# julienperriercornet/turbosqueeze

Hardware: AMD Instinct MI355X
Metric: encode+decode GB/s on enwik9-shaped input (round trip of uncompressed bytes) (higher is better)
Workload: dtype u8

## Files before the change

### turbosqueeze_amd/csrc/tsq_dec_common.cuh

```cuda
#pragma once

#include <type_traits>

#include "tsq_common.cuh"

namespace tsq {

#ifdef TSQ_STATS
__device__ unsigned long long g_dec_stats[16];
__device__ unsigned long long g_dec_wave[48];
#define TSQD_T0() unsigned long long t0_ = __builtin_amdgcn_s_memtime()
#define TSQD_ACC(slot) do { unsigned long long t1_ = __builtin_amdgcn_s_memtime(); st_[slot] += t1_ - t0_; t0_ = t1_; } while (0)
#define TSQD_CNT(slot, v) st_[slot] += (v)
#else
#define TSQD_T0() do {} while (0)
#define TSQD_ACC(slot) do {} while (0)
#define TSQD_CNT(slot, v) do {} while (0)
#endif

struct SymCfg {
    static constexpr uint32_t T = 1024;
    static constexpr uint32_t S = 6144;
    static constexpr uint32_t SPAD = 160;
    static constexpr uint32_t OUTC = 2 * S;
    static constexpr uint32_t HOP = 16;
    static constexpr uint32_t MAXG = 512;
    static constexpr uint32_t MAXSN = MAXG / HOP + 2;
    static constexpr uint32_t PER = S / T;
    static constexpr uint32_t TERM = S + SPAD;
    static constexpr uint32_t R = 65536 + OUTC + 64;
    static constexpr uint32_t RPAD = 64;
    static constexpr uint32_t SWORDS = (S + SPAD + 16) / 16;
};
static_assert(SymCfg::R % 16 == 0, "ring phase");
static_assert(SymCfg::OUTC == 12 * SymCfg::T, "twelve bytes per lane");
static_assert(SymCfg::S % SymCfg::T == 0 && SymCfg::SWORDS <= SymCfg::T, "lane counts");
static_assert(SymCfg::MAXG <= SymCfg::T / 2 && SymCfg::MAXG % SymCfg::HOP == 0 && SymCfg::MAXG >= SymCfg::S / 13 + 2 * SymCfg::HOP, "group table");
static_assert(4 * SymCfg::MAXG <= 2 * SymCfg::T, "at most two pairs per lane");

__device__ __forceinline__ void pair_lens(uint32_t sb, uint32_t cc, uint32_t ext, uint32_t& slen, uint32_t& olen)
{
    const uint32_t hi = sb >> 4, lo = sb & 15u;
    const uint32_t lit_hi = cc & 2u, lit_lo = cc & 1u;
    const uint32_t o_hi = (!lit_hi && ext && hi < 3u) ? (hi + 2u) << 4 : hi + 1u;
    const uint32_t o_lo = (!lit_lo && ext && lo < 3u) ? (lo + 2u) << 4 : lo + 1u;
    slen = 1u + (lit_hi ? hi + 1u : 2u) + (lit_lo ? lo + 1u : 2u);
    olen = o_hi + o_lo;
}

struct Image {
    uint32_t op, len, at;
    __device__ __forceinline__ uint32_t lead() const { return at & 3u; }
    __device__ __forceinline__ uint32_t a0() const { return at & ~3u; }
};

__device__ __forceinline__ uint4 prefetch_words(const uint8_t* in, uint32_t at, uint32_t av)
{
    using C = SymCfg;
    const uint32_t tid = threadIdx.x;
    const uint32_t lim = av < C::S + C::SPAD ? av : C::S + C::SPAD;
    uint4 w = make_uint4(0, 0, 0, 0);
    if (tid < C::SWORDS && (tid << 4) + 16u <= lim) __builtin_memcpy(&w, in + at + (tid << 4), 16);
    return w;
}
template <class L>
__device__ __forceinline__ void stage_words(uint8_t* lds, const uint8_t* in, uint32_t at, uint32_t av, uint4 pre)
{
    using C = SymCfg;
    const uint32_t tid = threadIdx.x;
    if (tid < C::SWORDS) {
        uint4 w = pre;
        const uint32_t lim = av < C::S + C::SPAD ? av : C::S + C::SPAD, o = tid << 4;
        if (o < lim && o + 16u > lim) {
            uint32_t b[4] = {0, 0, 0, 0};
            for (uint32_t k = 0; o + k < lim; ++k) b[k >> 2] |= (uint32_t)in[at + o + k] << (8u * (k & 3u));
            w = make_uint4(b[0], b[1], b[2], b[3]);
        }
        *reinterpret_cast<uint4*>(lds + L::sbuf + (tid << 4)) = w;
    }
}

template <class L>
__device__ __forceinline__ void parse_groups(uint8_t* lds, uint32_t slim, uint32_t (&x)[SymCfg::PER])
{
    using C = SymCfg;
    const uint32_t tid = threadIdx.x;
    const uint8_t* const sbuf = lds + L::sbuf;
    uint32_t y[C::PER], c[C::PER];
    {
        uint32_t* const pl = reinterpret_cast<uint32_t*>(lds + L::j4);
        constexpr uint32_t NW = (C::S + C::SPAD) / 4u;
#pragma unroll
        for (uint32_t k = 0; k < (NW + C::T - 1u) / C::T; ++k) {
            const uint32_t w = tid + k * C::T;
            if (w < NW) {
                const uint32_t v = reinterpret_cast<const uint32_t*>(sbuf)[w];
                uint32_t q[4];
#pragma unroll
                for (uint32_t b = 0; b < 4; ++b) {
                    const uint32_t hi = (v >> (8u * b + 4u)) & 15u, lo = (v >> (8u * b)) & 15u;
                    q[b] = 0x03040405u + (lo << 8) + (hi << 16) + ((lo + hi) << 24);
                }
                *reinterpret_cast<uint4*>(pl + 4u * w) = make_uint4(q[0], q[1], q[2], q[3]);
            }
        }
    }
    __syncthreads();
    {
        const uint32_t* const pl = reinterpret_cast<const uint32_t*>(lds + L::j4);
#pragma unroll
        for (uint32_t k = 0; k < C::PER; ++k) { const uint32_t o = tid + k * C::T; c[k] = (uint32_t)sbuf[o] << 3; x[k] = o + 1u; }
#pragma unroll
        for (uint32_t pr = 0; pr < 4; ++pr) {
#pragma unroll
            for (uint32_t k = 0; k < C::PER; ++k) y[k] = pl[x[k]];
#pragma unroll
            for (uint32_t k = 0; k < C::PER; ++k) x[k] += __builtin_amdgcn_ubfe(y[k], (c[k] >> (6u - 2u * pr)) & 0x18u, 8u);
        }
    }
    uint8_t* const j1 = lds + L::j1;
#pragma unroll
    for (uint32_t k = 0; k < C::PER; ++k) { const uint32_t o = tid + k * C::T; j1[o] = (uint8_t)(x[k] - o); x[k] = o < slim ? x[k] : C::TERM; }
    __syncthreads();
}

template <class L>
__device__ __forceinline__ void double_pointers(uint8_t* lds, uint32_t slim, uint32_t (&x)[SymCfg::PER])
{
    using C = SymCfg;
    const uint32_t tid = threadIdx.x;
    const uint8_t* const j1 = lds + L::j1;
    uint16_t* const j2 = reinterpret_cast<uint16_t*>(lds + L::j2);
    uint16_t* const j4 = reinterpret_cast<uint16_t*>(lds + L::j4);
    uint16_t* const j8 = reinterpret_cast<uint16_t*>(lds + L::j8);
    uint16_t* const j16 = reinterpret_cast<uint16_t*>(lds + L::j16);
    uint32_t y[C::PER];
#pragma unroll
    for (uint32_t k = 0; k < C::PER; ++k) { const uint32_t a = x[k] < slim ? x[k] : 0u; y[k] = a + j1[a]; }
#pragma unroll
    for (uint32_t k = 0; k < C::PER; ++k) { x[k] = x[k] < slim ? y[k] : C::TERM; j2[tid + k * C::T] = (uint16_t)x[k]; }
    if (tid <= C::SPAD) { j2[C::S + tid] = (uint16_t)C::TERM; j4[C::S + tid] = (uint16_t)C::TERM; j8[C::S + tid] = (uint16_t)C::TERM; j16[C::S + tid] = (uint16_t)C::TERM; }
    __syncthreads();
    const uint16_t* src = j2;
    uint16_t* const dsts[3] = {j4, j8, j16};
#pragma unroll
    for (uint32_t d = 0; d < 3; ++d) {
#pragma unroll
        for (uint32_t k = 0; k < C::PER; ++k) y[k] = src[x[k]];
#pragma unroll
        for (uint32_t k = 0; k < C::PER; ++k) { x[k] = y[k]; dsts[d][tid + k * C::T] = (uint16_t)x[k]; }
        __syncthreads();
        src = dsts[d];
    }
}

template <class L>
__device__ __forceinline__ uint32_t walk_chain(uint8_t* lds, uint32_t first, uint32_t slim)
{
    using C = SymCfg;
    const uint16_t* const j16 = reinterpret_cast<const uint16_t*>(lds + L::j16);
    uint16_t* const sn = reinterpret_cast<uint16_t*>(lds + L::sn);
    uint32_t* const misc = reinterpret_cast<uint32_t*>(lds + L::misc);
    if (threadIdx.x < 64u) {
        uint32_t x = first, k = 0;
        while (x < slim && k < C::MAXSN) {
            const uint32_t x1 = j16[x];
            const uint32_t x2 = j16[x1];
            sn[k++] = (uint16_t)x;
            if (x1 < slim && k < C::MAXSN) { sn[k++] = (uint16_t)x1; x = x2; }
            else x = x1;
        }
        if (threadIdx.x == 0) { misc[0] = k; if (k >= C::MAXSN && x < slim) misc[4] = kErrStream; }
    }
    __syncthreads();
    return misc[0];
}

template <class L>
__device__ __forceinline__ void group_lanes(uint8_t* lds, uint32_t nsn, uint32_t slim, uint32_t op, uint32_t size, uint32_t ext)
{
    using C = SymCfg;
    const uint32_t tid = threadIdx.x, lane = tid & 63u, wid = tid >> 6;
    const uint8_t* const sbuf = lds + L::sbuf;
    const uint8_t* const j1 = lds + L::j1;
    const uint16_t* const j2 = reinterpret_cast<const uint16_t*>(lds + L::j2);
    const uint16_t* const j4 = reinterpret_cast<const uint16_t*>(lds + L::j4);
    const uint16_t* const j8 = reinterpret_cast<const uint16_t*>(lds + L::j8);
    const uint16_t* const sn = reinterpret_cast<const uint16_t*>(lds + L::sn);
    uint16_t* const gstart = reinterpret_cast<uint16_t*>(lds + L::gstart);
    uint16_t* const glen = reinterpret_cast<uint16_t*>(lds + L::glen);
    uint32_t* const gout = reinterpret_cast<uint32_t*>(lds + L::gout);
    uint32_t* const pairs = reinterpret_cast<uint32_t*>(lds + L::pairs);
    uint32_t* const wsum = reinterpret_cast<uint32_t*>(lds + L::wsum);
    uint32_t* const misc = reinterpret_cast<uint32_t*>(lds + L::misc);
    uint32_t x = C::TERM;
    if (tid < nsn * C::HOP) {
        x = sn[tid >> 4];
        if (tid & 8u) x = j8[x];
        if (tid & 4u) x = j4[x];
        if (tid & 2u) x = j2[x];
        if (tid & 1u) x = x < slim ? (uint32_t)(x + j1[x]) : C::TERM;
    }
    uint32_t v = 0;
    if (x < slim) {
        gstart[tid] = (uint16_t)x;
        const uint32_t c = sbuf[x];
        uint32_t p = x + 1u, pw[4];
#pragma unroll
        for (uint32_t pr = 0; pr < 4; ++pr) {
            const uint32_t cc = (c >> (6u - 2u * pr)) & 3u;
            pw[pr] = p | (v << 13) | (cc << 30);
            uint32_t sl, ol;
            pair_lens(sbuf[p], cc, ext, sl, ol);
            p += sl;
            v += ol;
        }
        *reinterpret_cast<uint4*>(pairs + tid * 4u) = make_uint4(pw[0], pw[1], pw[2], pw[3]);
        glen[tid] = (uint16_t)v;
        if (p >= slim) { misc[1] = tid + 1u; misc[5] = p; }
    }
    const uint32_t incl = wave_scan_add(v);
    if (lane == 63) wsum[wid] = incl;
    __syncthreads();
    const uint32_t totals = wave_scan_add(lane < C::T / 64u ? wsum[lane] : 0u);
    const uint32_t before = wid ? (uint32_t)__builtin_amdgcn_readlane((int)totals, (int)wid - 1) : 0u;
    const uint32_t excl = before + incl - v;
    if (x < slim) {
        gout[tid] = op + excl;
        if (excl + 512u + 16u > C::OUTC) atomicMin(&misc[2], tid);
        if (op + excl + v >= size) atomicMin(&misc[3], tid);
    }
}

struct ChunkEnd {
    uint32_t ng;
    uint32_t next_at;
    uint32_t next_op;
    bool last;
    bool cut;
};
template <class L>
__device__ __forceinline__ ChunkEnd chunk_end(const uint8_t* lds, uint32_t op, uint32_t size)
{
    const uint16_t* const gstart = reinterpret_cast<const uint16_t*>(lds + L::gstart);
    const uint16_t* const glen = reinterpret_cast<const uint16_t*>(lds + L::glen);
    const uint32_t* const gout = reinterpret_cast<const uint32_t*>(lds + L::gout);
    const uint32_t* const misc = reinterpret_cast<const uint32_t*>(lds + L::misc);
    const uint32_t ng = misc[1], cut = misc[2], fin = misc[3];
    if (fin != 0xFFFFFFFFu && fin < cut) return {fin + 1u, 0u, size, true, false};
    if (cut != 0xFFFFFFFFu) return {cut, gstart[cut], gout[cut], false, true};
    return {ng, misc[5], ng ? gout[ng - 1] + glen[ng - 1] : op, false, false};
}

template <class L>
__device__ __forceinline__ void clear_records(uint8_t* lds)
{
    uint32_t* const recw = reinterpret_cast<uint32_t*>(lds + L::recw);
    for (uint32_t w = threadIdx.x; w < (SymCfg::OUTC + 16) / 4; w += SymCfg::T) *reinterpret_cast<uint4*>(recw + 4u * w) = make_uint4(0, 0, 0, 0);
}
template <class L, class PairAt>
__device__ __forceinline__ void drop_records(uint8_t* lds, uint32_t ng, const Image& im, uint32_t size, uint32_t avail, uint32_t ext,
                                             PairAt pair_at)
{
    using C = SymCfg;
    const uint32_t tid = threadIdx.x;
    const uint8_t* const sbuf = lds + L::sbuf;
    uint32_t* const recw = reinterpret_cast<uint32_t*>(lds + L::recw);
    const uint32_t op = im.op, lead = im.lead(), a0 = im.a0();
    if (tid == 0 && lead) recw[0] = 0x40000000u | (L::ring + a0);
    uint32_t bad = 0;
#pragma unroll
    for (uint32_t rep = 0; rep < 2; ++rep) {
        const uint32_t gi = tid + rep * C::T;
        if (gi >= ng * 4u) break;
        const uint2 pg = pair_at(rep, gi);
        const uint32_t pw = pg.x;
        uint32_t p = pw & 0x1FFFu, j = pg.y + ((pw >> 13) & 0x3FFFu);
        const uint32_t origin = j;
        uint32_t sb = 0;
        if (j < size) { if (p >= avail) bad = 1; sb = sbuf[p]; p++; }
#pragma unroll
        for (uint32_t sidx = 0; sidx < 2; ++sidx) {
            if (j < size && !bad) {
                const uint32_t nib = sidx == 0 ? sb >> 4 : sb & 15u;
                const uint32_t lit = (pw >> (31u - sidx)) & 1u;
                const uint32_t room = size - j;
                const uint32_t ij = j - op + lead;
                if (lit) {
                    const uint32_t len = nib + 1u, take = len < room ? len : room;
                    if (p + take > avail) bad = 1;
                    else recw[ij] = 0x40000000u | ((L::sbuf + p - ij) & 0xFFFFFFu);
                    p += len; j += take;
                } else {
                    if (p + 2u > avail) bad = 1;
                    const uint32_t off = (uint32_t)sbuf[p] | ((uint32_t)sbuf[p + 1] << 8);
                    p += 2;
                    const uint32_t len = ext ? nibble_span(nib) : nib + 1u;
                    const uint32_t take = len < room ? len : room;
                    if (off > origin || take > off) bad = 1;
                    if (!bad) {
                        const uint32_t a = origin - off;
                        const uint32_t n_hist = a >= op ? 0u : (op - a < take ? op - a : take);
                        if (n_hist) {
                            uint32_t x0 = a0 + C::R - ((op - a) - lead);
                            x0 -= x0 >= C::R ? C::R : 0u;
                            recw[ij] = 0x40000000u | ((L::ring + x0 - ij) & 0xFFFFFFu);
                            if (x0 + n_hist > C::R) { const uint32_t n1 = C::R - x0; recw[ij + n1] = 0x40000000u | ((L::ring - (ij + n1)) & 0xFFFFFFu); }
                        }
                        if (n_hist < take) recw[ij + n_hist] = 0xC0000000u | ((a - j) & 0xFFFFFFu);
                    }
                    j += take;
                }
            }
        }
    }
    if (bad) reinterpret_cast<uint32_t*>(lds + L::misc)[4] = kErrStream;
}

typedef __attribute__((address_space(3))) uint16_t lds_u16;

template <class L>
__device__ __forceinline__ uint32_t fetch_bytes(uint8_t* lds, const Image& im)
{
    const uint32_t tid = threadIdx.x, lane = tid & 63u, wid = tid >> 6;
    const uint32_t* const recw = reinterpret_cast<const uint32_t*>(lds + L::recw);
    uint32_t* const wsum = reinterpret_cast<uint32_t*>(lds + L::wsum);
    lds_u16* const wl = (lds_u16*)(lds + L::plist) + 768u * wid;
    const uint32_t own = 12u * tid;
    uint32_t r[12];
    {
        const uint4 q0 = *reinterpret_cast<const uint4*>(recw + own), q1 = *reinterpret_cast<const uint4*>(recw + own + 4u),
                    q2 = *reinterpret_cast<const uint4*>(recw + own + 8u);
        r[0] = q0.x; r[1] = q0.y; r[2] = q0.z; r[3] = q0.w; r[4] = q1.x; r[5] = q1.y; r[6] = q1.z; r[7] = q1.w; r[8] = q2.x; r[9] = q2.y; r[10] = q2.z; r[11] = q2.w;
#pragma unroll
        for (uint32_t k = 1; k < 12; ++k) r[k] = r[k] ? r[k] : r[k - 1];
        const uint32_t upto = wave_scan_last(r[11]);
        uint32_t carry = (uint32_t)__builtin_amdgcn_update_dpp(0, (int)upto, 0x138, 0xF, 0xF, false);
        if (lane == 63) wsum[wid] = upto;
        __syncthreads();
        {
            const uint32_t ws = lane < 16u ? wsum[lane] : 0u;
            const uint64_t m = __ballot(ws != 0u && lane < wid);
            const uint32_t prev = m ? (uint32_t)__builtin_amdgcn_readlane((int)ws, 63 - __builtin_clzll(m)) : 0u;
            carry = carry ? carry : prev;
        }
#pragma unroll
        for (uint32_t k = 0; k < 12; ++k) r[k] = r[k] ? r[k] : carry;
    }
    uint32_t pend = 0;
    if (own < im.lead() + im.len) {
        uint32_t v[12], by[12];
#pragma unroll
        for (uint32_t k = 0; k < 12; ++k) {
            v[k] = own + k + (uint32_t)((int32_t)(r[k] << 8) >> 8);
            pend |= (r[k] >> 31) << k;
        }
#pragma unroll
        for (uint32_t k = 0; k < 12; ++k) by[k] = lds[(r[k] >> 31) ? 0u : v[k]];
#pragma unroll
        for (uint32_t k = 0; k < 12; ++k) v[k] = (r[k] >> 31) ? v[k] : (0x8000u | by[k]);
#pragma unroll
        for (uint32_t w = 0; w < 3; ++w)
            *reinterpret_cast<uint2*>(lds + L::ent + 2u * own + 8u * w) = make_uint2(v[4 * w] | (v[4 * w + 1] << 16), v[4 * w + 2] | (v[4 * w + 3] << 16));
    }
    const uint32_t cnt = (uint32_t)__builtin_popcount(pend);
    const uint32_t incl = wave_scan_add(cnt);
    const uint32_t n_wait = (uint32_t)__builtin_amdgcn_readlane((int)incl, 63);
    uint32_t at = incl - cnt;
#pragma unroll
    for (uint32_t k = 0; k < 12; ++k) {
        if ((pend >> k) & 1u) wl[at] = (uint16_t)(own + k);
        at += (pend >> k) & 1u;
    }
    return n_wait;
}

template <class L>
__device__ __forceinline__ uint32_t jump_pointers(uint8_t* lds, uint32_t n_wait)
{
    const uint32_t lane = threadIdx.x & 63u, wid = threadIdx.x >> 6;
    lds_u16* const le = (lds_u16*)(lds + L::ent);
    lds_u16* const wl = (lds_u16*)(lds + L::plist) + 768u * wid;
    const uint32_t spare = SymCfg::OUTC + wid;
    if (lane == 0) le[spare] = 0x8000u;
    const uint32_t passes = (n_wait + 63u) >> 6;
    const uint32_t padded = passes <= 2u ? 2u : passes <= 4u ? 4u : passes <= 6u ? 6u : passes <= 8u ? 8u : 12u;
    if (passes) for (uint32_t it = n_wait + lane; it < padded * 64u; it += 64u) wl[it] = (uint16_t)spare;
    uint32_t iters = 0;
    auto jump = [&](auto passes_c) {
        constexpr uint32_t P = decltype(passes_c)::value;
        uint32_t q[P], ptr[P];
#pragma unroll
        for (uint32_t ps = 0; ps < P; ++ps) q[ps] = wl[ps * 64u + lane];
#pragma unroll
        for (uint32_t ps = 0; ps < P; ++ps) ptr[ps] = __hip_atomic_load(&le[q[ps]], __ATOMIC_RELAXED, __HIP_MEMORY_SCOPE_WORKGROUP);
        for (;;) {
            uint32_t e[P], open = 0;
#pragma unroll
            for (uint32_t ps = 0; ps < P; ++ps) e[ps] = __hip_atomic_load(&le[(ptr[ps] & 0x8000u) ? q[ps] : ptr[ps]], __ATOMIC_RELAXED, __HIP_MEMORY_SCOPE_WORKGROUP);
#pragma unroll
            for (uint32_t ps = 0; ps < P; ++ps) {
                __hip_atomic_store(&le[q[ps]], (uint16_t)e[ps], __ATOMIC_RELAXED, __HIP_MEMORY_SCOPE_WORKGROUP);
                ptr[ps] = e[ps];
                open |= (e[ps] & 0x8000u) ^ 0x8000u;
            }
            iters++;
            if (__ballot(open != 0u) == 0ull) break;
        }
    };
    if (passes == 0u) {}
    else if (passes <= 2u) jump(std::integral_constant<uint32_t, 2>{});
    else if (passes <= 4u) jump(std::integral_constant<uint32_t, 4>{});
    else if (passes <= 6u) jump(std::integral_constant<uint32_t, 6>{});
    else if (passes <= 8u) jump(std::integral_constant<uint32_t, 8>{});
    else jump(std::integral_constant<uint32_t, 12>{});
    return iters;
}

template <class L>
__device__ __forceinline__ void write_ring(uint8_t* lds, const Image& im)
{
    using C = SymCfg;
    const uint32_t own = 12u * threadIdx.x;
    if (own >= im.lead() + im.len) return;
    const uint2 e0 = *reinterpret_cast<const uint2*>(lds + L::ent + 2u * own), e1 = *reinterpret_cast<const uint2*>(lds + L::ent + 2u * own + 8u),
                e2 = *reinterpret_cast<const uint2*>(lds + L::ent + 2u * own + 16u);
    const uint32_t ev[6] = {e0.x, e0.y, e1.x, e1.y, e2.x, e2.y};
#pragma unroll
    for (uint32_t w = 0; w < 3; ++w) {
        uint32_t x = im.a0() + own + 4u * w; x -= x >= C::R ? C::R : 0u;
        const uint32_t lo = ev[2 * w], hi = ev[2 * w + 1];
        *reinterpret_cast<uint32_t*>(lds + L::ring + x) = (lo & 0xFFu) | ((lo >> 8) & 0xFF00u) | ((hi & 0xFFu) << 16) | ((hi >> 16) << 24);
    }
}

template <class L>
__device__ __forceinline__ void flush_image(const uint8_t* lds, uint8_t* out, const Image& im, uint32_t first_tid, uint32_t n_threads)
{
    using C = SymCfg;
    const uint32_t tid = threadIdx.x;
    const uint8_t* const ring = lds + L::ring;
    if (im.len == 0 || tid < first_tid) return;
    const uint32_t t = tid - first_tid;
    const uint32_t head = (16u - (im.at & 15u)) & 15u;
    const uint32_t hb = head < im.len ? head : im.len;
    if (t < hb) out[im.op + t] = ring[im.at + t];
    const uint32_t words = (im.len - hb) >> 4;
    uint32_t ra = im.at + hb; ra -= ra >= C::R ? C::R : 0u;
    for (uint32_t w = t; w < words; w += n_threads) {
        uint32_t a = ra + (w << 4); a -= a >= C::R ? C::R : 0u;
        *reinterpret_cast<uint4*>(out + im.op + hb + (w << 4)) = *reinterpret_cast<const uint4*>(ring + a);
    }
    const uint32_t tail_at = hb + (words << 4);
    if (t < im.len - tail_at) { uint32_t a = ra + (words << 4) + t; a -= a >= C::R ? C::R : 0u; out[im.op + tail_at + t] = ring[a]; }
}

template <class L>
__device__ __forceinline__ void flush_window(const uint8_t* lds, uint8_t* out, const Image& im, uint32_t lo, uint32_t hi, uint32_t first_tid,
                                             uint32_t n_threads)
{
    using C = SymCfg;
    const uint32_t a = im.op > lo ? im.op : lo, b = im.op + im.len < hi ? im.op + im.len : hi;
    if (a >= b) return;
    uint32_t at = im.at + (a - im.op); at -= at >= C::R ? C::R : 0u;
    flush_image<L>(lds, out, Image{a - lo, b - a, at}, first_tid, n_threads);
}

}
```

### turbosqueeze_amd/csrc/tsq_dec_duo.cuh

```cuda
#pragma once

#include "tsq_common.cuh"
#include "tsq_dec_common.cuh"
#include "tsq_dec_sym.cuh"

namespace tsq {

struct DuoCfg {
    static constexpr uint32_t SLOTS = 4;
    static constexpr uint32_t HDR = 8;
    static constexpr uint32_t REC_WORDS = ((HDR + 5 * SymCfg::MAXG) + 63u) & ~63u;
    static constexpr uint32_t FLAG_STRIDE = 64;
    static constexpr uint32_t kLast = 1, kError = 2;
    static constexpr uint32_t kAbort = 0xFFFFFFFFu;
    static constexpr uint32_t kSpinLimit = 1u << 24;
};

__device__ __forceinline__ uint32_t duo_load_acquire(const uint32_t* p) { return __hip_atomic_load(p, __ATOMIC_RELAXED, __HIP_MEMORY_SCOPE_AGENT); }
__device__ __forceinline__ void duo_acquire_fence() { __builtin_amdgcn_fence(__ATOMIC_ACQUIRE, "agent"); }
__device__ __forceinline__ void duo_store_release(uint32_t* p, uint32_t v) { __hip_atomic_store(p, v, __ATOMIC_RELEASE, __HIP_MEMORY_SCOPE_AGENT); }

template <uint32_t NP>
__device__ __forceinline__ void duo_parse(const uint8_t* __restrict__ in, uint32_t in_len, uint32_t size, uint32_t ext, uint32_t me,
                                          uint32_t* __restrict__ ring_g, uint32_t* __restrict__ flags, int32_t* __restrict__ status, uint8_t* lds,
                                          uint32_t spin_limit)
{
    using C = SymCfg;
    using L = SymLds;
    const uint32_t* const gout = reinterpret_cast<const uint32_t*>(lds + L::gout);
    const uint32_t* const pairs = reinterpret_cast<const uint32_t*>(lds + L::pairs);
    uint32_t* const misc = reinterpret_cast<uint32_t*>(lds + L::misc);
    const uint32_t tid = threadIdx.x;

    if (size == 0u) return;
    if (tid == 0) misc[4] = 0;
    uint32_t e_delta = 0, e_op = 0, e_rec = 0;
    bool e_known = me == 0u;
    uint32_t* const entry_in = flags + 8u + 8u * me;
    uint32_t* const entry_out = flags + 8u + 8u * ((me + 1u) % NP);
    uint32_t n_in = 0, n_out = 0;
    auto prefetch = [&](uint32_t q) {
        const uint64_t at = 3ull + (uint64_t)q * C::S;
        return at < in_len ? prefetch_words(in, (uint32_t)at, in_len - (uint32_t)at) : make_uint4(0, 0, 0, 0);
    };
    uint4 pre = prefetch(me);
    auto give_up = [&](uint32_t why) {
        if (tid == 0) {
            if (why == 2u) atomicMax(status, kErrStall);
            duo_store_release(flags + 32, DuoCfg::kAbort);
        }
    };
    __syncthreads();

    for (uint32_t k = me;; k += NP) {
        const uint64_t w64 = 3ull + (uint64_t)k * C::S;
        const bool beyond = w64 >= in_len;
        const uint32_t W = beyond ? in_len : (uint32_t)w64;
        const uint32_t avail = in_len - W;
        const uint32_t slim = avail < C::S ? avail : C::S;
        if (!beyond) {
            stage_words<L>(lds, in, W, avail, pre);
            pre = prefetch(k + NP);
            __syncthreads();
            uint32_t x[C::PER];
            parse_groups<L>(lds, slim, x);
            double_pointers<L>(lds, slim, x);
        }
        uint32_t delta, op, rec_no;
        if (e_known) { delta = e_delta; op = e_op; rec_no = e_rec; e_known = false; }
        else {
            if (tid == 0) {
                uint32_t why = 0, spins = 0;
                for (;;) {
                    if (duo_load_acquire(entry_in) > n_in) break;
                    if ((spins & 63u) == 63u && (duo_load_acquire(flags + 32) == DuoCfg::kAbort || __hip_atomic_load(status, __ATOMIC_RELAXED, __HIP_MEMORY_SCOPE_AGENT) != 0)) { why = 1; break; }
                    if (++spins > spin_limit) { why = 2; break; }
                    __builtin_amdgcn_s_sleep(1);
                }
                duo_acquire_fence();
                misc[6] = why;
                if (!why) { misc[7] = __builtin_nontemporal_load(entry_in + 1); misc[8] = __builtin_nontemporal_load(entry_in + 2); misc[9] = __builtin_nontemporal_load(entry_in + 3); }
            }
            __syncthreads();
            if (misc[6] != 0) { give_up(misc[6]); return; }
            n_in++;
            const uint32_t d = misc[7];
            if (d >> 16) return;
            delta = d & 0xFFFFu; op = misc[8]; rec_no = misc[9];
            __syncthreads();
        }
        if (beyond) {
            if (tid == 0) atomicMax(status, kErrStream);
        }
        for (;;) {
            if (tid == 0) { misc[0] = 0; misc[1] = 0; misc[2] = 0xFFFFFFFFu; misc[3] = 0xFFFFFFFFu; misc[5] = 0; }
            __syncthreads();
            const uint32_t nsn = walk_chain<L>(lds, delta, slim);
            group_lanes<L>(lds, nsn, slim, op, size, ext);
            __syncthreads();
            const ChunkEnd e = chunk_end<L>(lds, op, size);
            const uint32_t next_delta = e.last || e.cut ? e.next_at : e.next_at - C::S;
            const bool bad = beyond || misc[4] != 0 || e.ng == 0 || (!e.last && !e.cut && (slim < C::S || e.next_at < C::S || next_delta >= C::SPAD));
            if (!e.cut || bad) {
                const uint32_t fl = bad ? 2u : e.last ? 1u : 0u;
                if (NP == 1u) {
                    if (fl) {  } else { e_delta = next_delta; e_op = e.next_op; e_rec = rec_no + 1u; e_known = true; }
                } else {
                    if (tid == 0) {
                        __builtin_nontemporal_store((fl << 16) | next_delta, entry_out + 1);
                        __builtin_nontemporal_store(e.next_op, entry_out + 2);
                        __builtin_nontemporal_store(rec_no + 1u, entry_out + 3);
                        duo_store_release(entry_out, n_out + 1u);
                    }
                    n_out++;
                }
            }
            if (tid == 0) {
                uint32_t why = 0, spins = 0;
                for (;;) {
                    const uint32_t done = duo_load_acquire(flags + 32);
                    if (done == DuoCfg::kAbort || ((spins & 255u) == 255u && __hip_atomic_load(status, __ATOMIC_RELAXED, __HIP_MEMORY_SCOPE_AGENT) != 0)) { why = 1; break; }
                    if (rec_no - done < DuoCfg::SLOTS && (NP == 1u || duo_load_acquire(flags) == rec_no)) break;
                    if (++spins > spin_limit) { why = 2; break; }
                    __builtin_amdgcn_s_sleep(8);
                }
                duo_acquire_fence();
                misc[6] = why;
            }
            __syncthreads();
            if (misc[6] != 0) { give_up(misc[6]); return; }
            uint32_t* const rec = ring_g + (size_t)(rec_no % DuoCfg::SLOTS) * DuoCfg::REC_WORDS;
            if (!bad) {
                for (uint32_t w = tid; w < 4u * e.ng; w += C::T) rec[DuoCfg::HDR + w] = pairs[w];
                for (uint32_t w = tid; w < e.ng; w += C::T) rec[DuoCfg::HDR + 4u * C::MAXG + w] = gout[w];
            }
            if (tid == 0) {
                rec[0] = W; rec[1] = op; rec[2] = e.ng; rec[3] = e.next_op;
                rec[4] = (e.last ? DuoCfg::kLast : 0u) | (bad ? DuoCfg::kError : 0u);
                rec[5] = e.cut ? W : W + C::S;
            }
            asm volatile("s_waitcnt vmcnt(0)" ::: "memory");
            __syncthreads();
            if (tid == 0) duo_store_release(flags, rec_no + 1u);
            if (bad) { if (tid == 0) atomicMax(status, kErrStream); return; }
            if (e.last) return;
            if (!e.cut) break;
            delta = next_delta; op = e.next_op; rec_no++;
        }
    }
}

struct DuoCopyLds {
    static constexpr uint32_t sbuf = 0;
    static constexpr uint32_t recw = sbuf + 16 * SymCfg::SWORDS;
    static constexpr uint32_t ent = recw;
    static constexpr uint32_t plist = ent + 2 * (SymCfg::OUTC + 16);
    static constexpr uint32_t wsum = recw + 4 * (SymCfg::OUTC + 16);
    static constexpr uint32_t misc = wsum + 64;
    static constexpr uint32_t ring = (misc + 64 + 15) & ~15u;
    static constexpr uint32_t total = ring + SymCfg::R + SymCfg::RPAD;
    static_assert(recw % 16 == 0 && plist % 16 == 0 && plist + 2 * SymCfg::OUTC <= wsum, "records, byte entries and waiting lists");
};
static_assert(DuoCopyLds::total <= 160 * 1024 && SymLds::total <= 160 * 1024, "LDS budget");

__device__ __forceinline__ void duo_copy(const uint8_t* __restrict__ in, uint32_t in_len, uint32_t size, uint32_t ext, uint8_t* __restrict__ out,
                                         const uint32_t* __restrict__ ring_g, uint32_t* __restrict__ flags, int32_t* __restrict__ status, uint8_t* lds,
                                         uint32_t spin_limit)
{
    using C = SymCfg;
    using L = DuoCopyLds;
    uint32_t* const misc = reinterpret_cast<uint32_t*>(lds + L::misc);
    const uint32_t tid = threadIdx.x;
    const uint32_t oskew = (uint32_t)((uintptr_t)out & 15u);
    uint32_t ring_op = oskew;
    Image prev = {0, 0, 0};
    uint32_t k = 0, made_seen = 0;
    uint32_t hdr_n[6] = {0, 0, 0, 0, 0, 0}, pw_n[2] = {0, 0}, go_n[2] = {0, 0};
    bool have_next = false;
    if (size == 0u) return;
    if (tid == 0) { misc[4] = 0; }
    auto fetch_record = [&](const uint32_t* rec) {
#pragma unroll
        for (uint32_t q = 0; q < 6; ++q) hdr_n[q] = __builtin_nontemporal_load(rec + q);
#pragma unroll
        for (uint32_t rep = 0; rep < 2; ++rep) {
            const uint32_t gi = tid + rep * C::T;
            pw_n[rep] = rec[DuoCfg::HDR + gi];
            go_n[rep] = rec[DuoCfg::HDR + 4u * C::MAXG + (gi >> 2)];
        }
    };
    uint4 pre = prefetch_words(in, 3u, in_len - 3u);
    uint32_t pre_sp = 3u;
    __syncthreads();

    for (;;) {
        flush_image<L>(lds, out, prev, 0, C::T);
        if (made_seen <= k) {
            if (tid == 0) {
                uint32_t give_up = 0, spins = 0, made = 0;
                for (;;) {
                    made = duo_load_acquire(flags);
                    if (made > k) break;
                    if ((spins & 255u) == 255u && __hip_atomic_load(status, __ATOMIC_RELAXED, __HIP_MEMORY_SCOPE_AGENT) != 0) { give_up = 1; break; }
                    if (++spins > spin_limit) { give_up = 2; break; }
                    __builtin_amdgcn_s_sleep(1);
                }
                duo_acquire_fence();
                misc[6] = give_up; misc[7] = made;
            }
            __syncthreads();
            if (misc[6] != 0) {
                if (tid == 0) { duo_store_release(flags + 32, DuoCfg::kAbort); if (misc[6] == 2) atomicMax(status, kErrStall); }
                return;
            }
            made_seen = misc[7];
            have_next = false;
        }
        if (!have_next) fetch_record(ring_g + (size_t)(k % DuoCfg::SLOTS) * DuoCfg::REC_WORDS);
        const uint32_t sp = hdr_n[0], op = hdr_n[1], ng = hdr_n[2], next_op = hdr_n[3], flg = hdr_n[4], next_sp = hdr_n[5];
        have_next = false;
        if (flg & DuoCfg::kError) return;
        const bool last_chunk = (flg & DuoCfg::kLast) != 0u;
        const Image im = {op, next_op - op, ring_op};
        const uint32_t avail = in_len - sp;
        if (pre_sp != sp) pre = prefetch_words(in, sp, avail);
        stage_words<L>(lds, in, sp, avail, pre);
        clear_records<L>(lds);
        if (!last_chunk) { pre = prefetch_words(in, next_sp, in_len - next_sp); pre_sp = next_sp; }
        __syncthreads();

        drop_records<L>(lds, ng, im, size, avail, ext, [&](uint32_t rep, uint32_t) { return make_uint2(pw_n[rep], go_n[rep]); });
        __syncthreads();
        k++;
        if (misc[4] != 0) {
            if (tid == 0) { atomicMax(status, (int32_t)misc[4]); duo_store_release(flags + 32, DuoCfg::kAbort); }
            return;
        }
        if (tid == 0) __hip_atomic_store(flags + 32, k, __ATOMIC_RELAXED, __HIP_MEMORY_SCOPE_AGENT);
        if (!last_chunk && made_seen > k) {
            fetch_record(ring_g + (size_t)(k % DuoCfg::SLOTS) * DuoCfg::REC_WORDS);
            have_next = true;
        }
        const uint32_t n_wait = fetch_bytes<L>(lds, im);
        __syncthreads();
        jump_pointers<L>(lds, n_wait);
        __syncthreads();
        write_ring<L>(lds, im);
        prev = im;
        ring_op += im.len; ring_op -= ring_op >= C::R ? C::R : 0u;
        __syncthreads();
        if (last_chunk) break;
    }
    flush_image<L>(lds, out, prev, 0, C::T);
}

#ifdef TSQ_STATS
__device__ uint32_t g_duo_xcc[2048];
#endif
template <uint32_t NP>
__global__ __launch_bounds__(1024) void dec_duo_kernel(const uint8_t* __restrict__ container, const FrameInfo* __restrict__ frames, uint32_t n_blocks,
                                                       uint8_t* __restrict__ outbuf, int32_t* __restrict__ status,
                                                       uint32_t* __restrict__ ring_g, uint32_t* __restrict__ flags_g, uint32_t spin_limit)
{
    extern __shared__ __attribute__((aligned(16))) uint8_t lds[];
    const uint32_t w = blockIdx.x, xcd = w & 7u, slot = w >> 3;
    const uint32_t role = slot % (NP + 1u), b = (slot / (NP + 1u)) * 8u + xcd;
#ifdef TSQ_STATS
    if (threadIdx.x == 0 && w < 2048u) { uint32_t id; asm volatile("s_getreg_b32 %0, hwreg(HW_REG_XCC_ID)" : "=s"(id)); g_duo_xcc[w] = 0x80000000u | (id & 15u); }
#endif
    if (b >= n_blocks) return;
    {
        uint32_t* const seen = reinterpret_cast<uint32_t*>(lds);
        if (threadIdx.x == 0) seen[0] = (uint32_t)__hip_atomic_load(status, __ATOMIC_RELAXED, __HIP_MEMORY_SCOPE_AGENT);
        __syncthreads();
        const uint32_t st = seen[0];
        __syncthreads();
        if (st != 0u) return;
    }
    const FrameInfo f = frames[b];
    if (f.stream_len < 3u || f.stream_len > kSlotSize || f.out_len > kBlockSize) {
        if (threadIdx.x == 0) atomicMax(status, kErrStream);
        return;
    }
    uint32_t* const ring_b = ring_g + (size_t)b * DuoCfg::SLOTS * DuoCfg::REC_WORDS;
    uint32_t* const flags = flags_g + (size_t)b * DuoCfg::FLAG_STRIDE;
    if (role < NP) duo_parse<NP>(container + f.stream_at, f.stream_len, f.out_len, f.ext, role, ring_b, flags, status, lds, spin_limit);
    else duo_copy(container + f.stream_at, f.stream_len, f.out_len, f.ext, outbuf + f.out_at, ring_b, flags, status, lds, spin_limit);
}

}
```

### turbosqueeze_amd/csrc/tsq_dec_sym.cuh

```cuda
#pragma once

#include "tsq_common.cuh"
#include "tsq_dec_common.cuh"

namespace tsq {

struct SymLds {
    static constexpr uint32_t sbuf = 0;
    static constexpr uint32_t j1 = sbuf + 16 * SymCfg::SWORDS;
    static constexpr uint32_t JN = (SymCfg::S + SymCfg::SPAD + 8u) & ~7u;
    static constexpr uint32_t j2 = j1 + SymCfg::S;
    static constexpr uint32_t j4 = j2 + 2 * JN;
    static constexpr uint32_t j8 = j4 + 2 * JN;
    static constexpr uint32_t j16 = j8 + 2 * JN;
    static constexpr uint32_t recw = j1;
    static constexpr uint32_t ent = j1;
    static constexpr uint32_t plist = ent + 2 * (SymCfg::OUTC + 16);
    static constexpr uint32_t gstart = j16 + 2 * JN;
    static constexpr uint32_t glen = gstart + 2 * SymCfg::MAXG;
    static constexpr uint32_t gout = glen + 2 * SymCfg::MAXG;
    static constexpr uint32_t pairs = gout + 4 * SymCfg::MAXG;
    static constexpr uint32_t sn = pairs + 16 * SymCfg::MAXG;
    static constexpr uint32_t wsum = (sn + 2 * ((SymCfg::MAXSN + 7) & ~7u) + 15) & ~15u;
    static constexpr uint32_t misc = wsum + 64;
    static constexpr uint32_t ring = (misc + 64 + 15) & ~15u;
    static constexpr uint32_t total = ring + SymCfg::R + SymCfg::RPAD;
    static_assert(recw % 16 == 0 && recw + 4 * (SymCfg::OUTC + 16) <= gstart && plist % 16 == 0 && plist + 2 * SymCfg::OUTC <= gstart,
                  "records, byte entries and waiting lists fit the dead doubling tables");
};
static_assert(SymLds::total <= 160 * 1024, "LDS budget");

struct RangeItem {
    uint32_t block, lo, hi, pad;
    uint64_t out_at;
};

struct BlockGroup {
    uint32_t block, first, count, hi;
};

enum DecMode : int { kDecWhole, kDecWindow, kDecGroup };

struct GroupCursor {
    uint32_t cur = 0, cur_lo = 0;
    uint32_t held = 0xFFFFFFFFu;
    RangeItem it = {0u, 0u, 0u, 0u, 0ull};
};

template <class L>
__device__ __forceinline__ void flush_group(const uint8_t* lds, uint8_t* out, const Image& im, const RangeItem* items, uint32_t count, GroupCursor& gc,
                                            uint32_t first_tid, uint32_t n_threads)
{
    using C = SymCfg;
    const uint32_t tid = threadIdx.x;
    if (im.len == 0 || tid < first_tid || gc.cur >= count || gc.cur_lo >= im.op + im.len) return;
    uint32_t& cur = gc.cur;
    const uint8_t* const ring = lds + L::ring;
    const uint32_t lane = tid & 63u, w = (tid - first_tid) >> 6, nw = n_threads >> 6;
    const uint32_t im_end = im.op + im.len;
    uint32_t pass0 = 0;
    bool leading = true;
    for (uint32_t base = cur & ~63u; base < count; base += 64u) {
        const uint32_t k = base + lane;
        RangeItem it = {0u, 0xFFFFFFFFu, 0u, 0u, 0ull};
        if (base == gc.held) it = gc.it;
        else if (k < count) it = items[k];
        const bool in_run = it.lo < im_end;
        if (leading) {
            gc.held = base; gc.it = it;
            const uint64_t done = __ballot(k < count && it.hi <= im.op);
            const uint32_t n = ~done == 0ull ? 64u : (uint32_t)__builtin_ctzll(~done);
            cur = base + n;
            leading = n == 64u;
            if (!leading) gc.cur_lo = (uint32_t)__builtin_amdgcn_readlane((int)it.lo, (int)n);
        }
        const uint32_t a = it.lo > im.op ? it.lo : im.op, b = it.hi < im_end ? it.hi : im_end;
        const bool live = in_run && a < b;
        const uint32_t len = live ? b - a : 0u;
        const uint64_t addr = (uint64_t)(uintptr_t)out + it.out_at + (a - it.lo);
        const uint32_t nwords = live ? (((uint32_t)addr & 15u) + len + 15u) >> 4 : 0u;
        uint32_t ra = im.at + (a - im.op); ra -= ra >= C::R ? C::R : 0u;
        uint32_t incl = nwords;
#pragma unroll
        for (uint32_t d = 1; d < 64u; d <<= 1) {
            const uint32_t up = __shfl_up(incl, d);
            if (lane >= d) incl += up;
        }
        const uint32_t total = (uint32_t)__builtin_amdgcn_readlane((int)incl, 63);
        const uint32_t passes = (total + 63u) >> 6;
        const uint32_t packed = len | (ra << 14);
        for (uint32_t j = (w + nw - pass0 % nw) % nw; j < passes; j += nw) {
            const uint32_t q = (j << 6) + lane;
            uint32_t t = 0;
#pragma unroll
            for (uint32_t step = 32u; step != 0u; step >>= 1) {
                const uint32_t v = __shfl(incl, (int)(t + step - 1u));
                t += v <= q ? step : 0u;
            }
            const bool act = q < total;
            const int src = (int)(t & 63u);
            const uint32_t excl_s = __shfl(incl - nwords, src), alo = __shfl((uint32_t)addr, src), ahi = __shfl((uint32_t)(addr >> 32), src),
                           pk = __shfl(packed, src);
            if (act) {
                const uint32_t kk = q - excl_s, slen = pk & 0x3FFFu, sra = pk >> 14, s = alo & 15u;
                uint8_t* const word = reinterpret_cast<uint8_t*>((uintptr_t)((((uint64_t)ahi << 32) | alo) & ~15ull)) + ((size_t)kk << 4);
                const int32_t i0 = (int32_t)(kk << 4) - (int32_t)s;
                const uint32_t e0 = kk == 0u ? s : 0u;
                const uint32_t left = (uint32_t)((int32_t)slen - i0), e1 = left < 16u ? left : 16u;
                int32_t r = (int32_t)sra + i0;
                r += r < 0 ? (int32_t)C::R : 0; r -= r >= (int32_t)C::R ? (int32_t)C::R : 0;
                const uint32_t r0 = (uint32_t)r & ~15u;
                uint32_t r1 = r0 + 16u; r1 -= r1 >= C::R ? C::R : 0u;
                const uint4 x = *reinterpret_cast<const uint4*>(ring + r0), y = *reinterpret_cast<const uint4*>(ring + r1);
                const uint32_t v8[8] = {x.x, x.y, x.z, x.w, y.x, y.y, y.z, y.w};
                const uint32_t dsh = ((uint32_t)r >> 2) & 3u, bsh = ((uint32_t)r & 3u) << 3;
                uint32_t u[5], o[4];
#pragma unroll
                for (uint32_t i = 0; i < 5u; ++i) u[i] = dsh == 0u ? v8[i] : dsh == 1u ? v8[i + 1] : dsh == 2u ? v8[i + 2] : v8[i + 3];
#pragma unroll
                for (uint32_t i = 0; i < 4u; ++i) o[i] = (uint32_t)((((uint64_t)u[i + 1] << 32) | u[i]) >> bsh);
                if (e0 == 0u && e1 == 16u) {
                    *reinterpret_cast<uint4*>(word) = make_uint4(o[0], o[1], o[2], o[3]);
                } else {
#pragma unroll
                    for (uint32_t i = 0; i < 4u; ++i) {
                        if (e0 <= 4u * i && 4u * i + 4u <= e1) {
                            *reinterpret_cast<uint32_t*>(word + 4u * i) = o[i];
                        } else {
#pragma unroll
                            for (uint32_t c = 0; c < 4u; ++c)
                                if (4u * i + c >= e0 && 4u * i + c < e1) word[4u * i + c] = (uint8_t)(o[i] >> (8u * c));
                        }
                    }
                }
            }
        }
        pass0 += passes;
        if (__ballot(!in_run) != 0ull) break;
    }
}

template <DecMode kMode>
__device__ __forceinline__ void sym_decode_block(const uint8_t* container, const FrameInfo* frames, uint32_t n_frames, const RangeItem* items,
                                                 uint8_t* outbuf, int32_t* status, const BlockGroup* groups = nullptr, uint32_t n_items = 0u)
{
    constexpr bool kWindow = kMode == kDecWindow, kGroup = kMode == kDecGroup;
    using C = SymCfg;
    using L = SymLds;
    extern __shared__ __attribute__((aligned(16))) uint8_t lds[];
    const uint32_t* const gout = reinterpret_cast<const uint32_t*>(lds + L::gout);
    const uint32_t* const pairs = reinterpret_cast<const uint32_t*>(lds + L::pairs);
    uint32_t* const misc = reinterpret_cast<uint32_t*>(lds + L::misc);

    const uint32_t tid = threadIdx.x;
    if (tid == 0) misc[11] = (uint32_t)*status;
    __syncthreads();
    if (misc[11] != 0u) return;
    uint32_t blk = blockIdx.x, lo = 0, hi = 0;
    uint64_t out_at = 0;
    if constexpr (kWindow) {
        const RangeItem it = items[blockIdx.x];
        if (it.block >= n_frames) {
            if (tid == 0) atomicMax(status, kErrStream);
            return;
        }
        blk = it.block; lo = it.lo; hi = it.hi; out_at = it.out_at;
    }
    [[maybe_unused]] const RangeItem* gitems = nullptr;
    [[maybe_unused]] uint32_t gcount = 0;
    [[maybe_unused]] GroupCursor gcur;
    if constexpr (kGroup) {
        const BlockGroup g = groups[blockIdx.x];
        if (g.block >= n_frames || g.count == 0u || g.first > n_items || g.count > n_items - g.first) {
            if (tid == 0) atomicMax(status, kErrStream);
            return;
        }
        blk = g.block; hi = g.hi; gitems = items + g.first; gcount = g.count;
    }
    const FrameInfo f = frames[blk];
    if (f.stream_len < 3u || f.stream_len > kSlotSize || f.out_len > kBlockSize || ((kWindow || kGroup) && (lo >= hi || hi > f.out_len))) {
        if (tid == 0) atomicMax(status, kErrStream);
        return;
    }
    const uint8_t* const in = container + f.stream_at;
    uint8_t* const out = kGroup ? outbuf : outbuf + (kWindow ? out_at : f.out_at);
    const uint32_t in_len = f.stream_len, size = f.out_len, ext = f.ext;
    const uint32_t oskew = kGroup ? 0u : (uint32_t)(((uintptr_t)out - lo) & 15u);

#ifdef TSQ_STATS
    const uint32_t lane = tid & 63u, wid = tid >> 6;
    unsigned long long st_[16] = {0};
    unsigned long long wj_[3] = {0, 0, 0};
#endif
    TSQD_T0();
    if (tid == 0) { misc[4] = 0; misc[9] = 0; misc[10] = 0; }
    uint32_t sp = 3, op = 0;
    uint32_t ring_op = oskew;
    Image prev = {0, 0, 0};
    uint4 pre = prefetch_words(in, sp, in_len - sp);
    bool staged_ahead = false;
    __syncthreads();

    while (op < size) {
        const uint32_t avail = in_len - sp;
        const uint32_t slim = avail < C::S ? avail : C::S;
        if (!staged_ahead) stage_words<L>(lds, in, sp, avail, pre);
        if (tid == 0) { misc[0] = 0; misc[1] = 0; misc[2] = 0xFFFFFFFFu; misc[3] = 0xFFFFFFFFu; misc[5] = 0; }
        __syncthreads();
        TSQD_ACC(0); TSQD_CNT(12, 1);

        uint32_t x[C::PER];
        parse_groups<L>(lds, slim, x);
        TSQD_ACC(1);
        double_pointers<L>(lds, slim, x);
        TSQD_ACC(2);
        const uint32_t nsn = walk_chain<L>(lds, 0u, slim);
        TSQD_ACC(3);

        if (tid >= C::T / 2) {
            if constexpr (kGroup) flush_group<L>(lds, out, prev, gitems, gcount, gcur, C::T / 2, C::T / 2);
            else if constexpr (kWindow) flush_window<L>(lds, out, prev, lo, hi, C::T / 2, C::T / 2);
            else flush_image<L>(lds, out, prev, C::T / 2, C::T / 2);
        }
        group_lanes<L>(lds, nsn, slim, op, size, ext);
        clear_records<L>(lds);
        __syncthreads();
        const ChunkEnd e = chunk_end<L>(lds, op, size);
        const uint32_t next_sp = sp + e.next_at;
        if (misc[4] != 0 || e.ng == 0 || (!e.last && next_sp >= in_len)) {
            if (tid == 0) atomicMax(status, kErrStream);
            return;
        }
        const Image im = {op, e.next_op - op, ring_op};
        const bool more = !e.last && !((kWindow || kGroup) && e.next_op >= hi);
        if (more) pre = prefetch_words(in, next_sp, in_len - next_sp);
        TSQD_ACC(4);

        drop_records<L>(lds, e.ng, im, size, avail, ext,
                        [&](uint32_t, uint32_t gi) { return make_uint2(pairs[gi], gout[gi >> 2]); });
        __syncthreads();
        if (misc[4] != 0) { if (tid == 0) atomicMax(status, (int32_t)misc[4]); return; }
        TSQD_ACC(5);
        const uint32_t n_wait = fetch_bytes<L>(lds, im);
        __syncthreads();
        TSQD_ACC(6);
        if (more) { stage_words<L>(lds, in, next_sp, in_len - next_sp, pre); staged_ahead = true; }
#ifdef TSQ_STATS
        const unsigned long long wj0_ = __builtin_amdgcn_s_memtime();
#endif
        [[maybe_unused]] const uint32_t iters = jump_pointers<L>(lds, n_wait);
#ifdef TSQ_STATS
        if (lane == 0) { atomicMax(&misc[9], iters); atomicAdd(&misc[10], n_wait); }
        if (lane == 0 && blockIdx.x == 0) { wj_[0] += __builtin_amdgcn_s_memtime() - wj0_; wj_[1] += n_wait; wj_[2] += iters; }
#endif
        __syncthreads();
        write_ring<L>(lds, im);
        TSQD_ACC(7);
#ifdef TSQ_STATS
        if (tid == 0) { st_[14] += misc[9]; st_[11] += misc[10]; misc[9] = 0; misc[10] = 0; }
#endif

        prev = im;
        ring_op += im.len; ring_op -= ring_op >= C::R ? C::R : 0u;
        op = e.next_op;
        sp = next_sp;
        TSQD_ACC(8);
        if (!more) break;
    }
    if constexpr (kGroup) { if (tid == C::T / 2) misc[12] = gcur.cur; }
    __syncthreads();
    if constexpr (kGroup) { if (tid < C::T / 2) gcur.cur = misc[12]; }
    if constexpr (kGroup) flush_group<L>(lds, out, prev, gitems, gcount, gcur, 0, C::T);
    else if constexpr (kWindow) flush_window<L>(lds, out, prev, lo, hi, 0, C::T);
    else flush_image<L>(lds, out, prev, 0, C::T);
#ifdef TSQ_STATS
    if (blockIdx.x == 0 && tid == 0) for (int q = 0; q < 16; ++q) g_dec_stats[q] = st_[q];
    if (blockIdx.x == 0 && lane == 0) for (int q = 0; q < 3; ++q) g_dec_wave[wid * 3 + q] = wj_[q];
#endif
}

__global__ __launch_bounds__(1024) void dec_sym_kernel(const uint8_t* __restrict__ container, const FrameInfo* __restrict__ frames,
                                                       uint8_t* __restrict__ outbuf, int32_t* __restrict__ status)
{
    sym_decode_block<kDecWhole>(container, frames, 0u, nullptr, outbuf, status);
}

__global__ __launch_bounds__(1024) void dec_range_kernel(const uint8_t* __restrict__ container, const FrameInfo* __restrict__ frames, uint32_t n_frames,
                                                         const RangeItem* __restrict__ items, uint8_t* __restrict__ outbuf, int32_t* __restrict__ status)
{
    sym_decode_block<kDecWindow>(container, frames, n_frames, items, outbuf, status);
}

__global__ __launch_bounds__(1024) void dec_group_kernel(const uint8_t* __restrict__ container, const FrameInfo* __restrict__ frames, uint32_t n_frames,
                                                         const RangeItem* __restrict__ items, uint32_t n_items, const BlockGroup* __restrict__ groups,
                                                         uint8_t* __restrict__ outbuf, int32_t* __restrict__ status)
{
    sym_decode_block<kDecGroup>(container, frames, n_frames, items, outbuf, status, groups, n_items);
}

}
```

### turbosqueeze_amd/csrc/tsq_experiment.h

```cpp
#pragma once

#if defined(TSQ_X_NOHAZ) || defined(TSQ_X_NOCOMMITWAIT) || defined(TSQ_X_NOPATCH) || defined(TSQ_X_FAKE_TABLE) || defined(TSQ_X_FAKE_CAND) || \
    defined(TSQ_X_FREE_QUERY)
#define TSQ_TIMING_ONLY_BUILD 1
#ifndef TSQ_EXPERIMENT
#error "a timing-only switch (TSQ_X_*: wrong streams on purpose) needs -DTSQ_EXPERIMENT; the product library is never built with one (tools/xbuild.sh)"
#endif
#else
#define TSQ_TIMING_ONLY_BUILD 0
#endif

#if defined(TSQ_STATS) || defined(TSQ_SPINS) || defined(TSQ_TRACEONLY) || defined(TSQ_REGION) || defined(TSQ_JITTER) || defined(TSQ_X_DELAY_STAGE)
#define TSQ_INSTRUMENTED_BUILD 1
#else
#define TSQ_INSTRUMENTED_BUILD 0
#endif
```

### turbosqueeze_amd/csrc/tsq_launch.cuh

```cuda
#pragma once

#include <atomic>

#include "tsq_common.cuh"
#include "tsq_emit.cuh"
#include "tsq_internal.h"
#include "tsq_serial.cuh"
#include "tsq_dec_sym.cuh"
#include "tsq_dec_duo.cuh"
#include "tsq_enc_stage.cuh"
#ifdef TSQ_AB_VARIANTS
#include "ab/tsq_enc_stage_r05.cuh"
#endif

namespace tsq {

template <size_t N>
inline int raise_lds_limit(tsqa_ctx* c, std::atomic<uint64_t>& done, const void* const (&fns)[N], const uint32_t (&bytes)[N])
{
    const uint64_t dev_bit = 1ull << (c->device & 63);
    if (done.load() & dev_bit) return 0;
    for (size_t k = 0; k < N; ++k)
        if (hipFuncSetAttribute(fns[k], hipFuncAttributeMaxDynamicSharedMemorySize, (int)bytes[k]) != hipSuccess) {
            c->set_error("cannot reserve %u B of LDS", bytes[k]);
            return TSQA_ERR_HIP;
        }
    done.fetch_or(dev_bit);
    return 0;
}

#define TSQ_LAUNCH_ENC(KERNEL, THREADS, LDS)                                                                                        \
    hipLaunchKernelGGL((KERNEL), dim3(nb), dim3(THREADS), (LDS), s, in, (uint64_t)n, (uint64_t)readable, (uint64_t)stride, slots, sizes, c->tables, status)

inline int launch_encode_kernels(tsqa_ctx* c, const uint8_t* in, size_t n, size_t readable, size_t stride, uint32_t ext,
                                 uint8_t* slots, uint32_t* sizes, int32_t* status, hipStream_t s)
{
    const uint32_t nb = (uint32_t)((n + kBlockSize - 1) / kBlockSize);
    static std::atomic<uint64_t> attr_devices{0};
    {
        const void* const fns[4] = {reinterpret_cast<const void*>(enc_stage_kernel<true, true>), reinterpret_cast<const void*>(enc_stage_kernel<false, true>),
                                    reinterpret_cast<const void*>(enc_stage_kernel<true, false>), reinterpret_cast<const void*>(enc_stage_kernel<false, false>)};
        const uint32_t bytes[4] = {StageCfgT<true>::total, StageCfgT<true>::total, StageCfgT<false>::total, StageCfgT<false>::total};
        if (int rc = raise_lds_limit(c, attr_devices, fns, bytes)) return rc;
    }
    const int v = c->enc_variant;
    if (v == 1) {
        if (ext) TSQ_LAUNCH_ENC(enc_serial_kernel<true>, 64, 0);
        else     TSQ_LAUNCH_ENC(enc_serial_kernel<false>, 64, 0);
        return 0;
    }
#ifdef TSQ_AB_VARIANTS
    if (v == 5) {
        static std::atomic<uint64_t> ab_devices{0};
        const void* const fns[4] = {reinterpret_cast<const void*>(r05::enc_stage_kernel<true, true>), reinterpret_cast<const void*>(r05::enc_stage_kernel<false, true>),
                                    reinterpret_cast<const void*>(r05::enc_stage_kernel<true, false>), reinterpret_cast<const void*>(r05::enc_stage_kernel<false, false>)};
        const uint32_t bytes[4] = {r05::StageCfgT<true>::total, r05::StageCfgT<true>::total, r05::StageCfgT<false>::total, r05::StageCfgT<false>::total};
        if (int rc = raise_lds_limit(c, ab_devices, fns, bytes)) return rc;
        if (nb > (uint32_t)c->n_cus) {
            if (ext) TSQ_LAUNCH_ENC((r05::enc_stage_kernel<true, false>), r05::StageCfgT<false>::THREADS_LEAN, r05::StageCfgT<false>::total);
            else     TSQ_LAUNCH_ENC((r05::enc_stage_kernel<false, false>), r05::StageCfgT<false>::THREADS_LEAN, r05::StageCfgT<false>::total);
        } else {
            if (ext) TSQ_LAUNCH_ENC((r05::enc_stage_kernel<true, true>), r05::StageCfgT<true>::THREADS, r05::StageCfgT<true>::total);
            else     TSQ_LAUNCH_ENC((r05::enc_stage_kernel<false, true>), r05::StageCfgT<true>::THREADS, r05::StageCfgT<true>::total);
        }
        return 0;
    }
#else
    if (v == 5) { c->set_error("kernel variant %d lives in the A/B library only (make ab)", v); return TSQA_ERR_ARG; }
#endif
    if (v >= 2 && v <= 4) { c->set_error("kernel variant %d is not built", v); return TSQA_ERR_ARG; }
    const bool lean = v == 6 || (v == 0 && nb > (uint32_t)c->n_cus);
    if (lean) {
        if (ext) TSQ_LAUNCH_ENC((enc_stage_kernel<true, false>), StageCfgT<false>::THREADS_LEAN, StageCfgT<false>::total);
        else     TSQ_LAUNCH_ENC((enc_stage_kernel<false, false>), StageCfgT<false>::THREADS_LEAN, StageCfgT<false>::total);
    } else {
        if (ext) TSQ_LAUNCH_ENC((enc_stage_kernel<true, true>), StageCfgT<true>::THREADS, StageCfgT<true>::total);
        else     TSQ_LAUNCH_ENC((enc_stage_kernel<false, true>), StageCfgT<true>::THREADS, StageCfgT<true>::total);
    }
    return 0;
}
#undef TSQ_LAUNCH_ENC

#define TSQ_LAUNCH_BATCH(KERNEL, THREADS, LDS)                                                                                      \
    hipLaunchKernelGGL((KERNEL), dim3(nb), dim3(THREADS), (LDS), s, in, blocks, slots, sizes, c->tables, status)

inline int launch_batch_encode_kernels(tsqa_ctx* c, const uint8_t* in, const EncBatchBlock* blocks, uint32_t nb, uint32_t ext,
                                       uint8_t* slots, uint32_t* sizes, int32_t* status, hipStream_t s)
{
    static std::atomic<uint64_t> attr_devices{0};
    {
        const void* const fns[4] = {reinterpret_cast<const void*>(enc_batch_kernel<true, true>), reinterpret_cast<const void*>(enc_batch_kernel<false, true>),
                                    reinterpret_cast<const void*>(enc_batch_kernel<true, false>), reinterpret_cast<const void*>(enc_batch_kernel<false, false>)};
        const uint32_t bytes[4] = {StageCfgT<true>::total, StageCfgT<true>::total, StageCfgT<false>::total, StageCfgT<false>::total};
        if (int rc = raise_lds_limit(c, attr_devices, fns, bytes)) return rc;
    }
    const int v = c->enc_variant;
    if (v != 0 && v != 6 && v != 7) { c->set_error("kernel variant %d does not encode batches (0, 6 and 7 do)", v); return TSQA_ERR_ARG; }
    const bool lean = v == 6 || (v == 0 && nb > (uint32_t)c->n_cus);
    if (lean) {
        if (ext) TSQ_LAUNCH_BATCH((enc_batch_kernel<true, false>), StageCfgT<false>::THREADS_LEAN, StageCfgT<false>::total);
        else     TSQ_LAUNCH_BATCH((enc_batch_kernel<false, false>), StageCfgT<false>::THREADS_LEAN, StageCfgT<false>::total);
    } else {
        if (ext) TSQ_LAUNCH_BATCH((enc_batch_kernel<true, true>), StageCfgT<true>::THREADS, StageCfgT<true>::total);
        else     TSQ_LAUNCH_BATCH((enc_batch_kernel<false, true>), StageCfgT<true>::THREADS, StageCfgT<true>::total);
    }
    return 0;
}
#undef TSQ_LAUNCH_BATCH

inline int launch_decode_kernels(tsqa_ctx* c, const uint8_t* container, const FrameInfo* frames, uint32_t n_blocks, uint8_t* out,
                                 int32_t* status, hipStream_t s, int variant = -1)
{
    static std::atomic<uint64_t> attr_devices{0};
    {
        const void* const fns[1] = {reinterpret_cast<const void*>(dec_sym_kernel)};
        const uint32_t bytes[1] = {SymLds::total};
        if (int rc = raise_lds_limit(c, attr_devices, fns, bytes)) return rc;
    }
    const int v = variant >= 0 ? variant : c->dec_variant;
    if (v == 1) { hipLaunchKernelGGL(dec_serial_kernel, dim3(n_blocks), dim3(64), 0, s, container, frames, out, status); return 0; }
    if (v == 8 || v == 9) { c->set_error("kernel variant %d is not built", v); return TSQA_ERR_ARG; }
    auto launch_multi = [&](const FrameInfo* fr, uint32_t nblk, bool three) -> int {
        static std::atomic<uint64_t> duo_devices{0};
        const void* const fns[2] = {reinterpret_cast<const void*>(dec_duo_kernel<1>), reinterpret_cast<const void*>(dec_duo_kernel<2>)};
        const uint32_t lds_bytes = DuoCopyLds::total > SymLds::total ? DuoCopyLds::total : SymLds::total;
        const uint32_t bytes[2] = {lds_bytes, lds_bytes};
        if (int rc = raise_lds_limit(c, duo_devices, fns, bytes)) return rc;
        if (int rc = c->reserve_duo(nblk)) return rc;
        if (hipMemsetAsync(c->duo_flags, 0, (size_t)nblk * DuoCfg::FLAG_STRIDE * sizeof(uint32_t), s) != hipSuccess) { c->set_error("hipMemsetAsync failed"); return TSQA_ERR_HIP; }
        const uint32_t groups = (nblk + 7u) / 8u;
        if (three) hipLaunchKernelGGL(dec_duo_kernel<2>, dim3(24u * groups), dim3(SymCfg::T), lds_bytes, s, container, fr, nblk, out, status, c->duo_ring, c->duo_flags, c->decode_wait_limit);
        else hipLaunchKernelGGL(dec_duo_kernel<1>, dim3(16u * groups), dim3(SymCfg::T), lds_bytes, s, container, fr, nblk, out, status, c->duo_ring, c->duo_flags, c->decode_wait_limit);
        return 0;
    };
    const uint32_t cus = (uint32_t)c->n_cus;
    const bool trio = v == 5 || ((v == 0 || v == 3) && 3u * n_blocks <= cus);
    if (trio || v == 3 || v == 6 || (v == 0 && 2u * n_blocks <= cus)) return launch_multi(frames, n_blocks, trio && v != 6);
    if (v == 0 && n_blocks > cus) {
        const uint32_t tail = n_blocks % cus, full = n_blocks - tail;
        if (tail != 0u && 2u * tail <= cus) {
            hipLaunchKernelGGL(dec_sym_kernel, dim3(full), dim3(SymCfg::T), SymLds::total, s, container, frames, out, status);
            return launch_multi(frames + full, tail, 3u * tail <= cus);
        }
    }
    hipLaunchKernelGGL(dec_sym_kernel, dim3(n_blocks), dim3(SymCfg::T), SymLds::total, s, container, frames, out, status);
    return 0;
}

inline int launch_range_kernel(tsqa_ctx* c, const uint8_t* container, const FrameInfo* frames, uint32_t n_frames, const RangeItem* items,
                               uint32_t n_items, uint8_t* out, int32_t* status, hipStream_t s)
{
    static std::atomic<uint64_t> attr_devices{0};
    {
        const void* const fns[1] = {reinterpret_cast<const void*>(dec_range_kernel)};
        const uint32_t bytes[1] = {SymLds::total};
        if (int rc = raise_lds_limit(c, attr_devices, fns, bytes)) return rc;
    }
    hipLaunchKernelGGL(dec_range_kernel, dim3(n_items), dim3(SymCfg::T), SymLds::total, s, container, frames, n_frames, items, out, status);
    return 0;
}

inline int launch_group_kernel(tsqa_ctx* c, const uint8_t* container, const FrameInfo* frames, uint32_t n_frames, const RangeItem* items,
                               uint32_t n_items, const BlockGroup* groups, uint32_t n_groups, uint8_t* out, int32_t* status, hipStream_t s)
{
    static std::atomic<uint64_t> attr_devices{0};
    {
        const void* const fns[1] = {reinterpret_cast<const void*>(dec_group_kernel)};
        const uint32_t bytes[1] = {SymLds::total};
        if (int rc = raise_lds_limit(c, attr_devices, fns, bytes)) return rc;
    }
    hipLaunchKernelGGL(dec_group_kernel, dim3(n_groups), dim3(SymCfg::T), SymLds::total, s, container, frames, n_frames, items, n_items, groups, out, status);
    return 0;
}

}
```

### turbosqueeze_amd/csrc/tsq_runtime.hip

```cpp
#include "tsq_internal.h"

#include "tsq_batch.cuh"
#include "tsq_common.cuh"
#include "tsq_container.cuh"
#include "tsq_format.h"
#include "tsq_serial.cuh"
#include "tsq_launch.cuh"

#include <algorithm>
#include <cstdarg>
#include <cstdio>
#include <cstring>
#include <new>

using namespace tsq;

#define TSQ_HIP(ctx, call)                                                                       \
    do {                                                                                         \
        hipError_t e_ = (call);                                                                  \
        if (e_ != hipSuccess) {                                                                  \
            (ctx)->set_error("%s failed: %s", #call, hipGetErrorString(e_));                     \
            return TSQA_ERR_HIP;                                                                 \
        }                                                                                        \
    } while (0)

void tsqa_ctx::set_error(const char* fmt, ...)
{
    va_list ap;
    va_start(ap, fmt);
    vsnprintf(err, sizeof(err), fmt, ap);
    va_end(ap);
}

extern "C" size_t tsqa_block_count(size_t n) { return (n + kBlockSize - 1) / kBlockSize; }

extern "C" size_t tsqa_container_bound(size_t n) { return 16 + tsqa_block_count(n) * (size_t)(3 + kSlotSize); }

#define TSQ_STR2(x) #x
#define TSQ_STR(x) TSQ_STR2(x)
extern "C" const char* tsqa_build_info(void)
{
    return "arch=gfx950 timing_only=" TSQ_STR(TSQ_TIMING_ONLY_BUILD) " instrumented=" TSQ_STR(TSQ_INSTRUMENTED_BUILD)
#ifdef TSQ_AB_VARIANTS
           " ab_variants=1"
#else
           " ab_variants=0"
#endif
           " lm=" TSQ_STR(TSQ_LM) " lf=" TSQ_STR(TSQ_LF) " records=" TSQ_STR(TSQ_RECORDS) " [switches:"
#ifdef TSQ_X_NOHAZ
           " TSQ_X_NOHAZ"
#endif
#ifdef TSQ_X_NOCOMMITWAIT
           " TSQ_X_NOCOMMITWAIT"
#endif
#ifdef TSQ_X_NOPATCH
           " TSQ_X_NOPATCH"
#endif
#ifdef TSQ_X_FAKE_TABLE
           " TSQ_X_FAKE_TABLE"
#endif
#ifdef TSQ_X_FAKE_CAND
           " TSQ_X_FAKE_CAND"
#endif
#ifdef TSQ_X_FREE_QUERY
           " TSQ_X_FREE_QUERY"
#endif
#ifdef TSQ_X_DELAY_STAGE
           " TSQ_X_DELAY_STAGE"
#endif
#ifdef TSQ_STATS
           " TSQ_STATS"
#endif
#ifdef TSQ_SPINS
           " TSQ_SPINS"
#endif
#ifdef TSQ_TRACEONLY
           " TSQ_TRACEONLY"
#endif
#ifdef TSQ_JITTER
           " TSQ_JITTER"
#endif
#if !TSQ_TIMING_ONLY_BUILD && !TSQ_INSTRUMENTED_BUILD
           " none"
#endif
           "]";
}

extern "C" int tsqa_create(int device, tsqa_ctx** out)
{
    if (!out) return TSQA_ERR_ARG;
    *out = nullptr;
    int count = 0;
    if (hipGetDeviceCount(&count) != hipSuccess || count <= 0) return TSQA_ERR_NO_DEVICE;
    if (device < 0) { if (hipGetDevice(&device) != hipSuccess) return TSQA_ERR_NO_DEVICE; }
    if (device >= count) return TSQA_ERR_ARG;
    hipDeviceProp_t prop;
    if (hipGetDeviceProperties(&prop, device) != hipSuccess) return TSQA_ERR_NO_DEVICE;
    if (strncmp(prop.gcnArchName, "gfx950", 6) != 0) {
        fprintf(stderr, "turbosqueeze_amd: device %d is %s; this library carries gfx950 code only\n", device, prop.gcnArchName);
        return TSQA_ERR_NO_DEVICE;
    }
    tsqa_ctx* c = new (std::nothrow) tsqa_ctx();
    if (!c) return TSQA_ERR_ARG;
    c->device = device;
    c->n_cus = prop.multiProcessorCount;
    if (const char* e = getenv("TSQ_AMD_DECODE_WAIT_LIMIT")) { const long v = atol(e); if (v > 0) c->decode_wait_limit = (uint32_t)v; }
    if (hipSetDevice(device) != hipSuccess || hipStreamCreateWithFlags(&c->stream, hipStreamNonBlocking) != hipSuccess) {
        delete c;
        return TSQA_ERR_HIP;
    }
    if (hipMalloc(&c->d_size, sizeof(uint64_t)) != hipSuccess || hipMalloc(&c->d_status, sizeof(int32_t)) != hipSuccess) {
        tsqa_destroy(c);
        return TSQA_ERR_HIP;
    }
    *out = c;
    return TSQA_OK;
}

extern "C" void tsqa_destroy(tsqa_ctx* c)
{
    if (!c) return;
    (void)hipSetDevice(c->device);
    if (c->stream) { (void)hipStreamSynchronize(c->stream); (void)hipStreamDestroy(c->stream); }
    for (hipEvent_t e : c->prof_pool) if (e) (void)hipEventDestroy(e);
    (void)hipFree(c->slots); (void)hipFree(c->tables); (void)hipFree(c->sizes); (void)hipFree(c->frame_at);
    (void)hipFree(c->frames); (void)hipFree(c->d_size); (void)hipFree(c->d_status);
    (void)hipFree(c->duo_ring); (void)hipFree(c->duo_flags);
    if (c->host_frames) (void)hipHostFree(c->host_frames);
    if (c->host_frames_copied) (void)hipEventDestroy(c->host_frames_copied);
    for (tsqa_uploads* u : {&c->range_up, &c->batch_up})
        for (int k = 0; k < 2; ++k) {
            (void)hipFree(u->dev[k]);
            if (u->host[k]) (void)hipHostFree(u->host[k]);
            if (u->done[k]) (void)hipEventDestroy(u->done[k]);
        }
    (void)hipFree(c->batch_at); (void)hipFree(c->batch_sizes); (void)hipFree(c->batch_heads);
    delete c;
}

extern "C" const char* tsqa_last_error(const tsqa_ctx* c) { return c ? c->err : "null context"; }
extern "C" int tsqa_device_id(const tsqa_ctx* c) { return c ? c->device : -1; }
extern "C" void tsqa_set_kernel_variant(tsqa_ctx* c, int ev, int dv) { if (c) { c->enc_variant = ev; c->dec_variant = dv; } }
extern "C" void tsqa_set_decode_wait_limit(tsqa_ctx* c, uint32_t polls) { if (c) c->decode_wait_limit = polls ? polls : 1u; }

int tsqa_ctx::reserve(size_t n_blocks, bool want_tables, bool want_slots)
{
    (void)hipSetDevice(device);
    if (n_blocks > cap_blocks) {
        size_t nb = n_blocks;
        (void)hipStreamSynchronize(stream);
        (void)hipFree(sizes); (void)hipFree(frame_at); (void)hipFree(frames);
        sizes = nullptr; frame_at = nullptr; frames = nullptr; cap_blocks = 0;
        forget_sharded();
        TSQ_HIP(this, hipMalloc(&sizes, nb * sizeof(uint32_t)));
        TSQ_HIP(this, hipMalloc(&frame_at, (nb + 1) * sizeof(uint64_t)));
        TSQ_HIP(this, hipMalloc(&frames, nb * sizeof(FrameInfo)));
        cap_blocks = nb;
    }
    if (want_slots && n_blocks > cap_slots) {
        (void)hipStreamSynchronize(stream);
        (void)hipFree(slots); slots = nullptr; cap_slots = 0;
        TSQ_HIP(this, hipMalloc(&slots, n_blocks * (size_t)kSlotSize + 256));
        cap_slots = n_blocks;
    }
    if (want_tables && n_blocks > cap_tables) {
        (void)hipStreamSynchronize(stream);
        (void)hipFree(tables); tables = nullptr; cap_tables = 0;
        TSQ_HIP(this, hipMalloc(&tables, n_blocks * (size_t)kHashEntries * sizeof(uint16_t)));
        cap_tables = n_blocks;
    }
    return TSQA_OK;
}

int tsqa_ctx::reserve_duo(size_t n_blocks)
{
    (void)hipSetDevice(device);
    if (n_blocks <= cap_duo) return TSQA_OK;
    (void)hipStreamSynchronize(stream);
    (void)hipFree(duo_ring); (void)hipFree(duo_flags);
    duo_ring = nullptr; duo_flags = nullptr; cap_duo = 0;
    TSQ_HIP(this, hipMalloc(&duo_ring, n_blocks * (size_t)DuoCfg::SLOTS * DuoCfg::REC_WORDS * sizeof(uint32_t)));
    TSQ_HIP(this, hipMalloc(&duo_flags, n_blocks * (size_t)DuoCfg::FLAG_STRIDE * sizeof(uint32_t)));
    cap_duo = n_blocks;
    return TSQA_OK;
}

int tsqa_ctx::reserve_host_frames(size_t n)
{
    (void)hipSetDevice(device);
    if (host_frames_pending) { (void)hipEventSynchronize(host_frames_copied); host_frames_pending = false; }
    if (!host_frames_copied) TSQ_HIP(this, hipEventCreateWithFlags(&host_frames_copied, hipEventDisableTiming));
    if (n > cap_host_frames) {
        if (host_frames) (void)hipHostFree(host_frames);
        host_frames = nullptr; cap_host_frames = 0;
        size_t want = 64; while (want < n) want *= 2;
        TSQ_HIP(this, hipHostMalloc(reinterpret_cast<void**>(&host_frames), want * sizeof(FrameInfo), hipHostMallocDefault));
        cap_host_frames = want;
    }
    host_frame_src.resize(cap_host_frames);
    return TSQA_OK;
}

int tsqa_ctx::reserve_upload(tsqa_uploads& u, size_t bytes, int* slot)
{
    (void)hipSetDevice(device);
    const int k = u.next;
    u.next ^= 1;
    if (u.pending[k]) { (void)hipEventSynchronize(u.done[k]); u.pending[k] = false; }
    if (!u.done[k]) TSQ_HIP(this, hipEventCreateWithFlags(&u.done[k], hipEventDisableTiming));
    if (bytes > u.cap[k]) {
        if (u.host[k]) (void)hipHostFree(u.host[k]);
        (void)hipFree(u.dev[k]);
        u.host[k] = nullptr; u.dev[k] = nullptr; u.cap[k] = 0;
        size_t want = 4096; while (want < bytes) want *= 2;
        TSQ_HIP(this, hipHostMalloc(&u.host[k], want, hipHostMallocDefault));
        TSQ_HIP(this, hipMalloc(&u.dev[k], want));
        u.cap[k] = want;
    }
    *slot = k;
    return TSQA_OK;
}

int tsqa_ctx::reserve_batch(size_t n_items)
{
    (void)hipSetDevice(device);
    if (n_items <= cap_batch) return TSQA_OK;
    (void)hipStreamSynchronize(stream);
    (void)hipFree(batch_at); (void)hipFree(batch_sizes); (void)hipFree(batch_heads);
    batch_at = nullptr; batch_sizes = nullptr; batch_heads = nullptr; cap_batch = 0;
    size_t want = 256; while (want < n_items) want *= 2;
    TSQ_HIP(this, hipMalloc(&batch_at, want * sizeof(uint64_t)));
    TSQ_HIP(this, hipMalloc(&batch_sizes, want * sizeof(uint64_t)));
    TSQ_HIP(this, hipMalloc(&batch_heads, want * kHeaderSize));
    cap_batch = want;
    return TSQA_OK;
}

bool tsqa_ctx::prof_begin(int kind, hipStream_t s)
{
    if (!profiling || prof_used[kind] >= (uint32_t)kProfPairs) return false;
    const size_t at = ((size_t)kind * kProfPairs + prof_used[kind]) * 2;
    prof_used[kind]++;
    (void)hipEventRecord(prof_pool[at], s);
    return true;
}
void tsqa_ctx::prof_end(int kind, hipStream_t s)
{
    const size_t at = ((size_t)kind * kProfPairs + prof_used[kind] - 1) * 2 + 1;
    (void)hipEventRecord(prof_pool[at], s);
}

extern "C" int tsqa_profile_enable(tsqa_ctx* c, int on)
{
    if (!c) return TSQA_ERR_ARG;
    (void)hipSetDevice(c->device);
    if (on && c->prof_pool.empty()) {
        c->prof_pool.resize((size_t)tsqa_ctx::kProfKinds * tsqa_ctx::kProfPairs * 2, nullptr);
        for (auto& e : c->prof_pool)
            if (hipEventCreate(&e) != hipSuccess) {
                for (hipEvent_t made : c->prof_pool) if (made) (void)hipEventDestroy(made);
                c->prof_pool.clear();
                c->profiling = false;
                c->set_error("hipEventCreate failed");
                return TSQA_ERR_HIP;
            }
    }
    c->profiling = on != 0;
    return TSQA_OK;
}

static void drain_events(tsqa_ctx* c, int kind, double* ms, uint32_t* count)
{
    double sum = 0; uint32_t n = 0;
    for (uint32_t k = 0; k < c->prof_used[kind]; ++k) {
        const size_t at = ((size_t)kind * tsqa_ctx::kProfPairs + k) * 2;
        float t = 0;
        if (hipEventSynchronize(c->prof_pool[at + 1]) == hipSuccess && hipEventElapsedTime(&t, c->prof_pool[at], c->prof_pool[at + 1]) == hipSuccess) { sum += t; n++; }
    }
    c->prof_used[kind] = 0;
    if (ms) *ms = sum;
    if (count) *count = n;
}

extern "C" int tsqa_profile_read(tsqa_ctx* c, double* enc_ms, uint32_t* enc_n, double* dec_ms, uint32_t* dec_n)
{
    if (!c) return TSQA_ERR_ARG;
    (void)hipSetDevice(c->device);
    if (c->prof_pool.empty()) { if (enc_ms) *enc_ms = 0; if (enc_n) *enc_n = 0; if (dec_ms) *dec_ms = 0; if (dec_n) *dec_n = 0; return TSQA_OK; }
    drain_events(c, 0, enc_ms, enc_n);
    drain_events(c, 1, dec_ms, dec_n);
    return TSQA_OK;
}

extern "C" int tsqa_profile_read_calls(tsqa_ctx* c, double* comp_ms, uint32_t* comp_n, double* decomp_ms, uint32_t* decomp_n)
{
    if (!c) return TSQA_ERR_ARG;
    (void)hipSetDevice(c->device);
    if (c->prof_pool.empty()) { if (comp_ms) *comp_ms = 0; if (comp_n) *comp_n = 0; if (decomp_ms) *decomp_ms = 0; if (decomp_n) *decomp_n = 0; return TSQA_OK; }
    drain_events(c, 2, comp_ms, comp_n);
    drain_events(c, 3, decomp_ms, decomp_n);
    return TSQA_OK;
}


int tsqa_ctx::launch_encode_to(const void* d_in, size_t n, size_t readable, size_t stride, uint32_t ext, uint8_t* slots_out,
                               uint32_t* sizes_out, int32_t* status, hipStream_t s)
{
    const uint32_t nb = (uint32_t)tsqa_block_count(n);
    int rc = reserve(nb, true, false);
    if (rc) return rc;
    const bool timed = prof_begin(0, s);
    rc = launch_encode_kernels(this, static_cast<const uint8_t*>(d_in), n, readable, stride, ext, slots_out, sizes_out, status, s);
    if (rc) { if (timed) prof_used[0]--; return rc; }
    if (timed) prof_end(0, s);
    TSQ_HIP(this, hipGetLastError());
    return TSQA_OK;
}

int tsqa_ctx::launch_encode(const void* d_in, size_t n, size_t readable, uint32_t ext, int32_t* status, hipStream_t s)
{
    int rc = reserve((uint32_t)tsqa_block_count(n), true);
    if (rc) return rc;
    return launch_encode_to(d_in, n, readable, kBlockSize, ext, slots, sizes, status, s);
}

int tsqa_ctx::launch_pack(size_t n, uint32_t ext, void* d_out, size_t out_cap, uint64_t* d_out_size, int32_t* status, hipStream_t s)
{
    const uint32_t nb = (uint32_t)tsqa_block_count(n);
    hipLaunchKernelGGL(pack_scan_kernel, dim3(1), dim3(256), 0, s, sizes, nb, (uint64_t)n, ext,
                       static_cast<uint8_t*>(d_out), (uint64_t)out_cap, frame_at, d_out_size, status);
    const uint32_t pieces = (kSlotSize + kPackPiece - 1) / kPackPiece + 1;
    hipLaunchKernelGGL(pack_copy_kernel, dim3(pieces, nb), dim3(256), 0, s, slots, sizes, frame_at,
                       static_cast<uint8_t*>(d_out), status);
    TSQ_HIP(this, hipGetLastError());
    return TSQA_OK;
}

int tsqa_ctx::launch_decode_frames(const void* d_streams, const FrameInfo* d_frames, uint32_t n_blocks, void* d_out, int32_t* status, hipStream_t s, int variant)
{
    const bool timed = prof_begin(1, s);
    int rc = launch_decode_kernels(this, static_cast<const uint8_t*>(d_streams), d_frames, n_blocks, static_cast<uint8_t*>(d_out), status, s, variant);
    if (rc) { if (timed) prof_used[1]--; return rc; }
    if (timed) prof_end(1, s);
    TSQ_HIP(this, hipGetLastError());
    return TSQA_OK;
}

int tsqa_ctx::launch_decode(const void* d_container, uint32_t n_blocks, void* d_out, int32_t* status, hipStream_t s, int variant)
{
    return launch_decode_frames(d_container, frames, n_blocks, d_out, status, s, variant);
}

int tsqa_ctx::decode_again(const void* d_streams, const FrameInfo* d_frames, uint32_t n_blocks, void* d_out, int32_t* status, hipStream_t s)
{
    TSQ_HIP(this, hipMemsetAsync(status, 0, sizeof(int32_t), s));
    return launch_decode_frames(d_streams, d_frames, n_blocks, d_out, status, s, 4);
}


extern "C" int tsqa_compress_device_async(tsqa_ctx* c, const void* d_in, size_t n, void* d_out, size_t out_cap,
                                          uint64_t* d_out_size, int32_t* d_status, uint32_t ext, void* hip_stream)
{
    if (!c) return TSQA_ERR_ARG;
    if (!d_in || !d_out || !d_out_size || !d_status || n == 0) { c->set_error("compress: null pointer or zero size"); return TSQA_ERR_ARG; }
    if (out_cap < 16 + 6 * tsqa_block_count(n)) { c->set_error("compress: output capacity too small"); return TSQA_ERR_ARG; }
    hipStream_t s = hip_stream ? static_cast<hipStream_t>(hip_stream) : c->stream;
    (void)hipSetDevice(c->device);
    TSQ_HIP(c, hipMemsetAsync(d_status, 0, sizeof(int32_t), s));
    const bool timed = c->prof_begin(2, s);
    int rc = c->launch_encode(d_in, n, n, ext, d_status, s);
    if (rc) { if (timed) c->prof_used[2]--; return rc; }
    rc = c->launch_pack(n, ext, d_out, out_cap, d_out_size, d_status, s);
    if (timed) c->prof_end(2, s);
    return rc;
}

static int status_to_rc(tsqa_ctx* c, int32_t st, const char* what)
{
    if (st == 0) return TSQA_OK;
    c->set_error("%s: device reported status %d", what, st);
    return st;
}

extern "C" int tsqa_compress_device(tsqa_ctx* c, const void* d_in, size_t n, void* d_out, size_t out_cap,
                                    size_t* out_size, uint32_t ext, void* hip_stream)
{
    if (!c || !out_size) return TSQA_ERR_ARG;
    hipStream_t s = hip_stream ? static_cast<hipStream_t>(hip_stream) : c->stream;
    int rc = tsqa_compress_device_async(c, d_in, n, d_out, out_cap, c->d_size, c->d_status, ext, s);
    if (rc) return rc;
    uint64_t sz = 0; int32_t st = 0;
    TSQ_HIP(c, hipMemcpyAsync(&sz, c->d_size, sizeof(sz), hipMemcpyDeviceToHost, s));
    TSQ_HIP(c, hipMemcpyAsync(&st, c->d_status, sizeof(st), hipMemcpyDeviceToHost, s));
    TSQ_HIP(c, hipStreamSynchronize(s));
    *out_size = (size_t)sz;
    return status_to_rc(c, st, "compress");
}

static int decompress_device_async_impl(tsqa_ctx* c, const void* d_in, size_t n, uint32_t n_blocks, void* d_out,
                                        size_t out_cap, uint64_t* d_out_size, int32_t* d_status, void* hip_stream, int variant)
{
    if (!c) return TSQA_ERR_ARG;
    if (!d_in || !d_out || !d_out_size || !d_status || n < 16 || n_blocks == 0) { c->set_error("decompress: bad argument"); return TSQA_ERR_ARG; }
    hipStream_t s = hip_stream ? static_cast<hipStream_t>(hip_stream) : c->stream;
    (void)hipSetDevice(c->device);
    int rc = c->reserve(n_blocks, false, false);
    if (rc) return rc;
    c->forget_sharded();
    TSQ_HIP(c, hipMemsetAsync(d_status, 0, sizeof(int32_t), s));
    const bool timed = c->prof_begin(3, s);
    hipLaunchKernelGGL(frame_walk_kernel, dim3(1), dim3(64), 0, s, static_cast<const uint8_t*>(d_in), (uint64_t)n, n_blocks,
                       (uint64_t)out_cap, c->frames, d_out_size, d_status);
    rc = c->launch_decode(d_in, n_blocks, d_out, d_status, s, variant);
    if (timed) c->prof_end(3, s);
    return rc;
}

extern "C" int tsqa_decompress_device_async(tsqa_ctx* c, const void* d_in, size_t n, uint32_t n_blocks, void* d_out,
                                            size_t out_cap, uint64_t* d_out_size, int32_t* d_status, void* hip_stream)
{
    return decompress_device_async_impl(c, d_in, n, n_blocks, d_out, out_cap, d_out_size, d_status, hip_stream, -1);
}


extern "C" int tsqa_encode_blocks_async(tsqa_ctx* c, const void* d_in, uint32_t n_blocks, size_t stride, uint32_t last_len,
                                        uint32_t ext, void* d_slots, uint32_t* d_sizes, int32_t* d_status, void* hip_stream)
{
    if (!c) return TSQA_ERR_ARG;
    if (!d_in || !d_slots || !d_sizes || !d_status || n_blocks == 0 || last_len == 0 || last_len > kBlockSize || stride < kBlockSize) {
        c->set_error("encode_blocks: bad argument");
        return TSQA_ERR_ARG;
    }
    hipStream_t s = hip_stream ? static_cast<hipStream_t>(hip_stream) : c->stream;
    (void)hipSetDevice(c->device);
    TSQ_HIP(c, hipMemsetAsync(d_status, 0, sizeof(int32_t), s));
    const size_t n = (size_t)(n_blocks - 1) * kBlockSize + last_len;
    const size_t tail = stride > kBlockSize ? (stride - kBlockSize < 128 ? stride - kBlockSize : 128) : 0;
    const size_t readable = (size_t)(n_blocks - 1) * stride + last_len + tail;
    return c->launch_encode_to(d_in, n, readable, stride, ext, static_cast<uint8_t*>(d_slots), d_sizes, d_status, s);
}

extern "C" int tsqa_decode_blocks_async(tsqa_ctx* c, const void* d_streams, const tsqa_frame* d_frames, uint32_t n_blocks,
                                        void* d_out, int32_t* d_status, void* hip_stream)
{
    if (!c) return TSQA_ERR_ARG;
    if (!d_streams || !d_frames || !d_out || !d_status || n_blocks == 0) { c->set_error("decode_blocks: bad argument"); return TSQA_ERR_ARG; }
    static_assert(sizeof(tsqa_frame) == sizeof(FrameInfo), "public frame descriptor = kernel frame descriptor");
    hipStream_t s = hip_stream ? static_cast<hipStream_t>(hip_stream) : c->stream;
    (void)hipSetDevice(c->device);
    TSQ_HIP(c, hipMemsetAsync(d_status, 0, sizeof(int32_t), s));
    return c->launch_decode_frames(d_streams, reinterpret_cast<const FrameInfo*>(d_frames), n_blocks, d_out, d_status, s);
}

extern "C" int tsqa_decompress_device(tsqa_ctx* c, const void* d_in, size_t n, void* d_out, size_t out_cap,
                                      size_t* out_size, void* hip_stream)
{
    if (!c || !out_size) return TSQA_ERR_ARG;
    if (!d_in || n < 16) { c->set_error("decompress: bad argument"); return TSQA_ERR_ARG; }
    hipStream_t s = hip_stream ? static_cast<hipStream_t>(hip_stream) : c->stream;
    (void)hipSetDevice(c->device);
    uint8_t head[kHeaderSize];
    TSQ_HIP(c, hipMemcpyAsync(head, d_in, kHeaderSize, hipMemcpyDeviceToHost, s));
    TSQ_HIP(c, hipStreamSynchronize(s));
    uint32_t nb = 0; uint64_t total = 0;
    const int h = read_header(head, n, &nb, &total);
    if (h == kHeaderBadMagic || h == kHeaderNoBlocks) { c->set_error("decompress: bad magic or no blocks"); return TSQA_ERR_FORMAT; }
    if (total > out_cap) { c->set_error("decompress: output capacity %zu < %llu", out_cap, (unsigned long long)total); return TSQA_ERR_ARG; }
    if (h != kHeaderOk) { *out_size = 0; c->set_error("decompress: more blocks or bytes than a container of %zu B can hold", n); return TSQA_ERR_FORMAT; }
    int rc = tsqa_decompress_device_async(c, d_in, n, nb, d_out, out_cap, c->d_size, c->d_status, s);
    if (rc) return rc;
    uint64_t sz = 0; int32_t st = 0;
    TSQ_HIP(c, hipMemcpyAsync(&sz, c->d_size, sizeof(sz), hipMemcpyDeviceToHost, s));
    TSQ_HIP(c, hipMemcpyAsync(&st, c->d_status, sizeof(st), hipMemcpyDeviceToHost, s));
    TSQ_HIP(c, hipStreamSynchronize(s));
    if (st == kErrStall) {
        rc = decompress_device_async_impl(c, d_in, n, nb, d_out, out_cap, c->d_size, c->d_status, s, 4);
        if (rc) return rc;
        TSQ_HIP(c, hipMemcpyAsync(&sz, c->d_size, sizeof(sz), hipMemcpyDeviceToHost, s));
        TSQ_HIP(c, hipMemcpyAsync(&st, c->d_status, sizeof(st), hipMemcpyDeviceToHost, s));
        TSQ_HIP(c, hipStreamSynchronize(s));
    }
    *out_size = (size_t)sz;
    return status_to_rc(c, st, "decompress");
}

extern "C" int tsqa_frames_to_host_async(tsqa_ctx* c, const void* d_slots, const uint32_t* sizes, const uint64_t* frame_at,
                                         uint32_t n_blocks, uint32_t ext, void* host_container, void* hip_stream)
{
    if (!c) return TSQA_ERR_ARG;
    if (!d_slots || !sizes || !frame_at || !host_container) { c->set_error("frames_to_host: null pointer"); return TSQA_ERR_ARG; }
    hipStream_t s = hip_stream ? static_cast<hipStream_t>(hip_stream) : c->stream;
    (void)hipSetDevice(c->device);
    uint8_t* base = static_cast<uint8_t*>(host_container);
    for (uint32_t b = 0; b < n_blocks; ++b) {
        if (!stream_len_ok(sizes[b])) { c->set_error("frames_to_host: block %u has size %u", b, sizes[b]); return TSQA_ERR_ARG; }
        uint8_t* p = base + frame_at[b];
        write_frame(p, sizes[b], ext);
        TSQ_HIP(c, hipMemcpyAsync(p + kFrameWordSize, static_cast<const uint8_t*>(d_slots) + (size_t)b * kSlotSize, sizes[b], hipMemcpyDeviceToHost, s));
    }
    return TSQA_OK;
}

extern "C" int tsqa_frames_from_host_async(tsqa_ctx* c, const void* host_container, const uint64_t* frame_at, const uint32_t* sizes,
                                           uint32_t n_blocks, void* d_streams, void* hip_stream)
{
    if (!c) return TSQA_ERR_ARG;
    if (!d_streams || !sizes || !frame_at || !host_container) { c->set_error("frames_from_host: null pointer"); return TSQA_ERR_ARG; }
    hipStream_t s = hip_stream ? static_cast<hipStream_t>(hip_stream) : c->stream;
    (void)hipSetDevice(c->device);
    const uint8_t* base = static_cast<const uint8_t*>(host_container);
    for (uint32_t b = 0; b < n_blocks; ++b) {
        if (!stream_len_ok(sizes[b])) { c->set_error("frames_from_host: block %u has size %u", b, sizes[b]); return TSQA_ERR_FORMAT; }
        TSQ_HIP(c, hipMemcpyAsync(static_cast<uint8_t*>(d_streams) + (size_t)b * kSlotSize, base + frame_at[b] + kFrameWordSize, sizes[b], hipMemcpyHostToDevice, s));
    }
    return TSQA_OK;
}

extern "C" int tsqa_frame_offsets(const uint32_t* sizes, uint32_t n_blocks, uint64_t* frame_at, uint64_t* container_size)
{
    if (!sizes || !frame_at || !container_size) return TSQA_ERR_ARG;
    uint64_t at = kHeaderSize;
    for (uint32_t b = 0; b < n_blocks; ++b) {
        if (!stream_len_ok(sizes[b])) return TSQA_ERR_ARG;
        frame_at[b] = at;
        at += kFrameWordSize + (uint64_t)sizes[b];
    }
    *container_size = at;
    return TSQA_OK;
}

template <class Visit>
static int walk_host_frames(const uint8_t* p, size_t size, uint32_t nb, uint64_t total, const char** why, Visit&& visit)
{
    uint64_t at = kHeaderSize, sum = 0;
    for (uint32_t b = 0; b < nb; ++b) {
        FrameInfo f;
        if (at + kMinFrameSize > size || !read_frame(p + at, at, size, &f)) { *why = "malformed or truncated frame"; return TSQA_ERR_FORMAT; }
        if (!visit(b, at, f)) return TSQA_ERR_FORMAT;
        sum += f.out_len;
        at += kFrameWordSize + f.stream_len;
    }
    if (sum != total) { *why = "block sizes do not add up to the total"; return TSQA_ERR_FORMAT; }
    return TSQA_OK;
}

extern "C" int tsqa_walk_frames(const void* container, size_t size, uint32_t cap_blocks, uint64_t* frame_at, uint32_t* sizes, uint32_t* ext,
                                uint32_t* out_len, uint32_t* n_blocks, uint64_t* total)
{
    if (!container || !frame_at || !sizes || !ext || !out_len || !n_blocks || !total) return TSQA_ERR_ARG;
    const uint8_t* p = static_cast<const uint8_t*>(container);
    uint32_t nb; uint64_t tot;
    if (read_header(p, size, &nb, &tot) != kHeaderOk || nb > cap_blocks) return TSQA_ERR_FORMAT;
    const char* why;
    const int rc = walk_host_frames(p, size, nb, tot, &why, [&](uint32_t b, uint64_t at, const FrameInfo& f) {
        frame_at[b] = at; sizes[b] = f.stream_len; ext[b] = f.ext; out_len[b] = f.out_len;
        return true;
    });
    if (rc) return rc;
    *n_blocks = nb; *total = tot;
    return TSQA_OK;
}

extern "C" int tsqa_sharded_place_async(tsqa_ctx* c, const void* d_slots, const uint32_t* all_sizes, uint32_t n_blocks, uint64_t n_total,
                                        uint32_t rank, uint32_t world, uint32_t ext, void* host_container, size_t host_cap,
                                        uint64_t* container_size, void* hip_stream)
{
    if (!c) return TSQA_ERR_ARG;
    if (!d_slots || !all_sizes || !host_container || !container_size || world == 0 || rank >= world || n_blocks == 0) { c->set_error("sharded_place: bad argument"); return TSQA_ERR_ARG; }
    hipStream_t s = hip_stream ? static_cast<hipStream_t>(hip_stream) : c->stream;
    (void)hipSetDevice(c->device);
    uint8_t* base = static_cast<uint8_t*>(host_container);
    uint64_t at = kHeaderSize;
    for (uint32_t b = 0; b < n_blocks; ++b) {
        const uint32_t sz = all_sizes[b];
        if (!stream_len_ok(sz)) { c->set_error("sharded_place: block %u has size %u", b, sz); return TSQA_ERR_ARG; }
        at += kFrameWordSize + (uint64_t)sz;
    }
    if (at > host_cap) { c->set_error("sharded_place: the host container is too small (%llu > %zu)", (unsigned long long)at, host_cap); return TSQA_ERR_ARG; }
    at = kHeaderSize;
    for (uint32_t b = 0; b < n_blocks; ++b) {
        const uint32_t sz = all_sizes[b];
        if (b % world == rank) {
            write_frame(base + at, sz, ext);
            TSQ_HIP(c, hipMemcpyAsync(base + at + kFrameWordSize, static_cast<const uint8_t*>(d_slots) + (size_t)(b / world) * kSlotSize, sz, hipMemcpyDeviceToHost, s));
        }
        at += kFrameWordSize + (uint64_t)sz;
    }
    if (rank == 0) write_header(base, n_blocks, n_total);
    *container_size = at;
    return TSQA_OK;
}

extern "C" int tsqa_sharded_fetch_decode_async(tsqa_ctx* c, const void* host_container, size_t container_size, uint32_t rank, uint32_t world,
                                               void* d_streams, size_t streams_cap, void* d_out, size_t out_cap, int32_t* d_status, uint64_t* total,
                                               void* hip_stream)
{
    if (!c) return TSQA_ERR_ARG;
    if (!host_container || !d_streams || !d_out || !d_status || !total || world == 0 || rank >= world) { c->set_error("sharded_fetch_decode: bad argument"); return TSQA_ERR_ARG; }
    hipStream_t s = hip_stream ? static_cast<hipStream_t>(hip_stream) : c->stream;
    (void)hipSetDevice(c->device);
    const uint8_t* p = static_cast<const uint8_t*>(host_container);
    c->forget_sharded();
    uint32_t nb; uint64_t tot;
    if (read_header(p, container_size, &nb, &tot) != kHeaderOk) { c->set_error("sharded_fetch_decode: bad header"); return TSQA_ERR_FORMAT; }
    const uint32_t n_local = nb > rank ? (nb - rank + world - 1) / world : 0;
    if ((uint64_t)n_local * kSlotSize > streams_cap) { c->set_error("sharded_fetch_decode: %u owned frames do not fit d_streams (%zu B)", n_local, streams_cap); return TSQA_ERR_FORMAT; }
    if (int rc = c->reserve(n_local ? n_local : 1, false, false)) return rc;
    if (int rc = c->reserve_host_frames(n_local ? n_local : 1)) return rc;
    const char* why;
    const int rc = walk_host_frames(p, container_size, nb, tot, &why, [&](uint32_t b, uint64_t at, FrameInfo f) {
        if (b % world != rank) return true;
        const uint32_t k = b / world;
        if ((uint64_t)k * kBlockSize + f.out_len > out_cap) { why = "an owned block does not fit d_out"; return false; }
        f.stream_at = (uint64_t)k * kSlotSize; f.out_at = (uint64_t)k * kBlockSize;
        c->host_frames[k] = f;
        c->host_frame_src[k] = at + kFrameWordSize;
        return true;
    });
    if (rc) { c->set_error("sharded_fetch_decode: %s", why); return rc; }
    *total = tot;
    TSQ_HIP(c, hipMemsetAsync(d_status, 0, sizeof(int32_t), s));
    if (n_local == 0) return TSQA_OK;
    for (uint32_t k = 0; k < n_local; ++k)
        TSQ_HIP(c, hipMemcpyAsync(static_cast<uint8_t*>(d_streams) + (size_t)k * kSlotSize, p + c->host_frame_src[k], c->host_frames[k].stream_len, hipMemcpyHostToDevice, s));
    TSQ_HIP(c, hipMemcpyAsync(c->frames, c->host_frames, (size_t)n_local * sizeof(FrameInfo), hipMemcpyHostToDevice, s));
    TSQ_HIP(c, hipEventRecord(c->host_frames_copied, s));
    c->host_frames_pending = true;
    c->sharded_n_local = n_local; c->sharded_streams = d_streams; c->sharded_out = d_out;
    return c->launch_decode_frames(d_streams, c->frames, n_local, d_out, d_status, s);
}

extern "C" int tsqa_sharded_decode_again_async(tsqa_ctx* c, const void* d_streams, void* d_out, int32_t* d_status, void* hip_stream)
{
    if (!c) return TSQA_ERR_ARG;
    if (!d_streams || !d_out || !d_status) { c->set_error("sharded_decode_again: null pointer"); return TSQA_ERR_ARG; }
    if (c->sharded_n_local == 0) { c->set_error("sharded_decode_again: no sharded decode to repeat on this context (none yet, or another call has used the context since)"); return TSQA_ERR_ARG; }
    if (d_streams != c->sharded_streams || d_out != c->sharded_out) { c->set_error("sharded_decode_again: not the buffers of the sharded decode being repeated"); return TSQA_ERR_ARG; }
    hipStream_t s = hip_stream ? static_cast<hipStream_t>(hip_stream) : c->stream;
    (void)hipSetDevice(c->device);
    return c->decode_again(d_streams, c->frames, c->sharded_n_local, d_out, d_status, s);
}


extern "C" int tsqa_index_create(tsqa_ctx* c, const void* d_container, size_t n, tsqa_index** out)
{
    if (!out) return TSQA_ERR_ARG;
    *out = nullptr;
    if (!c) return TSQA_ERR_ARG;
    if (!d_container) { c->set_error("index_create: null container"); return TSQA_ERR_ARG; }
    if (n < kHeaderSize) { c->set_error("index_create: a container of %zu B has no header", n); return TSQA_ERR_FORMAT; }
    (void)hipSetDevice(c->device);
    hipStream_t s = c->stream;
    uint8_t head[kHeaderSize];
    TSQ_HIP(c, hipMemcpyAsync(head, d_container, kHeaderSize, hipMemcpyDeviceToHost, s));
    TSQ_HIP(c, hipStreamSynchronize(s));
    uint32_t nb; uint64_t total;
    if (read_header(head, n, &nb, &total) != kHeaderOk) { c->set_error("index_create: bad header"); return TSQA_ERR_FORMAT; }
    tsqa_index* idx = new (std::nothrow) tsqa_index();
    if (!idx) { c->set_error("index_create: out of host memory"); return TSQA_ERR_ARG; }
    idx->device = c->device; idx->container = static_cast<const uint8_t*>(d_container); idx->n = n; idx->n_blocks = nb; idx->total = total;
    int rc = TSQA_OK;
    int32_t st = 0;
    try {
        idx->host_frames.resize(nb);
        idx->out_start.resize((size_t)nb + 1);
    } catch (...) { rc = TSQA_ERR_ARG; c->set_error("index_create: out of host memory"); }
    auto walk = [&]() -> int {
        TSQ_HIP(c, hipMalloc(&idx->frames, (size_t)nb * sizeof(FrameInfo)));
        TSQ_HIP(c, hipMemsetAsync(c->d_status, 0, sizeof(int32_t), s));
        hipLaunchKernelGGL(frame_walk_kernel, dim3(1), dim3(64), 0, s, idx->container, (uint64_t)n, nb, total, idx->frames, c->d_size, c->d_status);
        TSQ_HIP(c, hipGetLastError());
        TSQ_HIP(c, hipMemcpyAsync(&st, c->d_status, sizeof(st), hipMemcpyDeviceToHost, s));
        TSQ_HIP(c, hipMemcpyAsync(idx->host_frames.data(), idx->frames, (size_t)nb * sizeof(FrameInfo), hipMemcpyDeviceToHost, s));
        TSQ_HIP(c, hipStreamSynchronize(s));
        return TSQA_OK;
    };
    if (rc == TSQA_OK) rc = walk();
    if (rc == TSQA_OK && st != 0) { c->set_error("index_create: malformed container (status %d)", st); rc = TSQA_ERR_FORMAT; }
    if (rc != TSQA_OK) { tsqa_index_destroy(idx); return rc; }
    for (uint32_t b = 0; b < nb; ++b) idx->out_start[b] = idx->host_frames[b].out_at;
    idx->out_start[nb] = total;
    try { idx->item_first = {0ull, (uint64_t)nb}; idx->item_status = {TSQA_OK}; }
    catch (...) { c->set_error("index_create: out of host memory"); tsqa_index_destroy(idx); return TSQA_ERR_ARG; }
    *out = idx;
    return TSQA_OK;
}

extern "C" void tsqa_index_destroy(tsqa_index* idx)
{
    if (!idx) return;
    (void)hipSetDevice(idx->device);
    (void)hipFree(idx->frames);
    delete idx;
}

extern "C" uint32_t tsqa_index_blocks(const tsqa_index* idx) { return idx ? idx->n_blocks : 0u; }
extern "C" uint64_t tsqa_index_total(const tsqa_index* idx) { return idx ? idx->total : 0ull; }
extern "C" uint32_t tsqa_index_items(const tsqa_index* idx) { return idx ? (uint32_t)idx->item_status.size() : 0u; }
extern "C" uint64_t tsqa_index_item_total(const tsqa_index* idx, uint32_t i)
{
    if (!idx || i >= idx->item_status.size()) return 0ull;
    return idx->out_start[idx->item_first[i + 1]] - idx->out_start[idx->item_first[i]];
}
extern "C" int tsqa_index_item_status(const tsqa_index* idx, uint32_t i)
{
    return idx && i < idx->item_status.size() ? idx->item_status[i] : TSQA_ERR_ARG;
}

static int plan_ranges(const uint64_t* out_start, uint32_t nb, const tsqa_range* r, uint32_t nr, size_t out_cap, tsqa_range_item* items,
                       uint32_t cap_items, uint32_t* n_items, const char** why, bool count_only = false)
{
    *why = "";
    if (!out_start || !n_items || (nr && !r) || nb == 0) { *why = "null pointer or no blocks"; return TSQA_ERR_ARG; }
    if (out_start[0] != 0) { *why = "out_start[0] is not 0"; return TSQA_ERR_ARG; }
    for (uint32_t b = 0; b < nb; ++b)
        if (out_start[b + 1] < out_start[b] || out_start[b + 1] - out_start[b] > kBlockSize) { *why = "a block is longer than TSQ_BLOCK_SZ"; return TSQA_ERR_ARG; }
    const uint64_t total = out_start[nb];
    auto first_block = [&](uint64_t at) -> uint32_t { return (uint32_t)(std::upper_bound(out_start, out_start + nb + 1, at) - out_start) - 1u; };
    std::vector<std::pair<uint64_t, uint64_t>> dst;
    uint64_t count = 0;
    for (uint32_t k = 0; k < nr; ++k) {
        const tsqa_range& x = r[k];
        if (x.length == 0) continue;
        if (x.length > total || x.offset > total - x.length) { *why = "a range ends past the total"; return TSQA_ERR_ARG; }
        if (x.length > out_cap || x.out_at > out_cap - x.length) { *why = "a range does not fit the output"; return TSQA_ERR_ARG; }
        dst.emplace_back(x.out_at, x.length);
        const uint64_t end = x.offset + x.length;
        for (uint32_t b = first_block(x.offset); b < nb && out_start[b] < end; ++b) count += out_start[b + 1] > out_start[b];
    }
    std::sort(dst.begin(), dst.end());
    for (size_t k = 1; k < dst.size(); ++k)
        if (dst[k - 1].first + dst[k - 1].second > dst[k].first) { *why = "the destinations of two ranges overlap"; return TSQA_ERR_ARG; }
    if (count > 0xFFFFFFFFull) { *why = "more than 2^32 - 1 items"; return TSQA_ERR_ARG; }
    *n_items = (uint32_t)count;
    if (count_only) return TSQA_OK;
    if (count > cap_items) { *why = "the items do not fit cap_items"; return TSQA_ERR_ARG; }
    uint32_t m = 0;
    for (uint32_t k = 0; k < nr; ++k) {
        const tsqa_range& x = r[k];
        if (x.length == 0) continue;
        const uint64_t end = x.offset + x.length;
        for (uint32_t b = first_block(x.offset); b < nb && out_start[b] < end; ++b) {
            const uint64_t a = x.offset > out_start[b] ? x.offset : out_start[b], e = end < out_start[b + 1] ? end : out_start[b + 1];
            if (a >= e) continue;
            items[m++] = tsqa_range_item{b, (uint32_t)(a - out_start[b]), (uint32_t)(e - out_start[b]), 0u, x.out_at + (a - x.offset)};
        }
    }
    return TSQA_OK;
}

extern "C" int tsqa_plan_ranges(const uint64_t* out_start, uint32_t n_blocks, const tsqa_range* ranges, uint32_t n_ranges, size_t out_cap,
                                tsqa_range_item* items, uint32_t cap_items, uint32_t* n_items)
{
    const char* why;
    if (!items && cap_items) return TSQA_ERR_ARG;
    return plan_ranges(out_start, n_blocks, ranges, n_ranges, out_cap, items, cap_items, n_items, &why);
}

extern "C" int tsqa_decompress_ranges_async(tsqa_ctx* c, const tsqa_index* idx, const tsqa_range* ranges, uint32_t n_ranges, void* d_out,
                                            size_t out_cap, int32_t* d_status, void* hip_stream)
{
    static_assert(sizeof(tsqa_range_item) == sizeof(RangeItem), "public range item = kernel range item");
    if (!c) return TSQA_ERR_ARG;
    if (!idx || !d_out || !d_status || (n_ranges && !ranges)) { c->set_error("decompress_ranges: null pointer"); return TSQA_ERR_ARG; }
    if (idx->device != c->device) { c->set_error("decompress_ranges: the index belongs to device %d, the context to %d", idx->device, c->device); return TSQA_ERR_ARG; }
    const char* why;
    uint32_t n_items = 0;
    if (plan_ranges(idx->out_start.data(), idx->n_blocks, ranges, n_ranges, out_cap, nullptr, 0, &n_items, &why, true)) {
        c->set_error("decompress_ranges: %s", why);
        return TSQA_ERR_ARG;
    }
    hipStream_t s = hip_stream ? static_cast<hipStream_t>(hip_stream) : c->stream;
    (void)hipSetDevice(c->device);
    int k = 0;
    if (int rc = c->reserve_upload(c->range_up, (size_t)(n_items ? n_items : 1) * sizeof(tsqa_range_item), &k)) return rc;
    tsqa_range_item* const host_items = static_cast<tsqa_range_item*>(c->range_up.host[k]);
    if (plan_ranges(idx->out_start.data(), idx->n_blocks, ranges, n_ranges, out_cap, host_items, (uint32_t)(c->range_up.cap[k] / sizeof(tsqa_range_item)), &n_items, &why)) {
        c->set_error("decompress_ranges: %s", why);
        return TSQA_ERR_ARG;
    }
    TSQ_HIP(c, hipMemsetAsync(d_status, 0, sizeof(int32_t), s));
    if (n_items == 0) return TSQA_OK;
    TSQ_HIP(c, hipMemcpyAsync(c->range_up.dev[k], host_items, (size_t)n_items * sizeof(tsqa_range_item), hipMemcpyHostToDevice, s));
    const int rc = launch_range_kernel(c, idx->container, idx->frames, idx->n_blocks, static_cast<const RangeItem*>(c->range_up.dev[k]),
                                       n_items, static_cast<uint8_t*>(d_out), d_status, s);
    TSQ_HIP(c, hipEventRecord(c->range_up.done[k], s));
    c->range_up.pending[k] = true;
    if (rc) return rc;
    TSQ_HIP(c, hipGetLastError());
    return TSQA_OK;
}

extern "C" int tsqa_decompress_ranges(tsqa_ctx* c, const tsqa_index* idx, const tsqa_range* ranges, uint32_t n_ranges, void* d_out,
                                      size_t out_cap, void* hip_stream)
{
    if (!c) return TSQA_ERR_ARG;
    hipStream_t s = hip_stream ? static_cast<hipStream_t>(hip_stream) : c->stream;
    int rc = tsqa_decompress_ranges_async(c, idx, ranges, n_ranges, d_out, out_cap, c->d_status, s);
    if (rc) return rc;
    int32_t st = 0;
    TSQ_HIP(c, hipMemcpyAsync(&st, c->d_status, sizeof(st), hipMemcpyDeviceToHost, s));
    TSQ_HIP(c, hipStreamSynchronize(s));
    return status_to_rc(c, st, "decompress_ranges");
}


static int plan_item_ranges(const uint64_t* out_start, uint32_t nb, const uint64_t* item_first, uint32_t n_items, const tsqa_item_range* r,
                            uint32_t nr, size_t out_cap, std::vector<tsqa_range_item>& items, std::vector<tsqa_block_group>& groups,
                            const char** why)
{
    *why = "";
    items.clear(); groups.clear();
    if (!out_start || !item_first || n_items == 0 || (nr && !r)) { *why = "null pointer or no items"; return TSQA_ERR_ARG; }
    if (item_first[0] != 0 || item_first[n_items] != nb) { *why = "item_first does not run from 0 to n_blocks"; return TSQA_ERR_ARG; }
    for (uint32_t i = 0; i < n_items; ++i)
        if (item_first[i + 1] < item_first[i]) { *why = "item_first decreases"; return TSQA_ERR_ARG; }
    uint32_t n = 0;
    if (nb && plan_ranges(out_start, nb, nullptr, 0, out_cap, nullptr, 0, &n, why, true)) return TSQA_ERR_ARG;
    std::vector<tsqa_range> flat;
    flat.reserve(nr);
    for (uint32_t k = 0; k < nr; ++k) {
        const tsqa_item_range& x = r[k];
        if (x.item >= n_items) { *why = "an item number past the index"; return TSQA_ERR_ARG; }
        const uint64_t fb = item_first[x.item], fe = item_first[x.item + 1];
        if (fb == fe) { *why = "a range of a refused item"; return TSQA_ERR_ARG; }
        const uint64_t total = out_start[fe] - out_start[fb];
        if (x.length > total || x.offset > total - x.length) { *why = "a range ends past its item's total"; return TSQA_ERR_ARG; }
        if (x.length) flat.push_back(tsqa_range{out_start[fb] + x.offset, x.length, x.out_at});
    }
    if (flat.empty()) return TSQA_OK;
    if (plan_ranges(out_start, nb, flat.data(), (uint32_t)flat.size(), out_cap, nullptr, 0, &n, why, true)) return TSQA_ERR_ARG;
    items.resize(n);
    if (plan_ranges(out_start, nb, flat.data(), (uint32_t)flat.size(), out_cap, items.data(), n, &n, why)) return TSQA_ERR_ARG;
    std::stable_sort(items.begin(), items.end(), [](const tsqa_range_item& p, const tsqa_range_item& q) {
        return p.block != q.block ? p.block < q.block : p.lo < q.lo;
    });
    for (uint32_t k = 0; k < n; ++k) {
        if (groups.empty() || groups.back().block != items[k].block) groups.push_back(tsqa_block_group{items[k].block, k, 0u, 0u});
        tsqa_block_group& g = groups.back();
        g.count++;
        g.hi = std::max(g.hi, items[k].hi);
    }
    return TSQA_OK;
}

extern "C" int tsqa_plan_item_ranges(const uint64_t* out_start, uint32_t n_blocks, const uint64_t* item_first_block, uint32_t n_items,
                                     const tsqa_item_range* ranges, uint32_t n_ranges, size_t out_cap, tsqa_range_item* items,
                                     uint32_t cap_items, uint32_t* n_range_items, tsqa_block_group* groups, uint32_t cap_groups,
                                     uint32_t* n_groups)
{
    const char* why;
    if (!n_range_items || !n_groups || (!items && cap_items) || (!groups && cap_groups)) return TSQA_ERR_ARG;
    std::vector<tsqa_range_item> vi;
    std::vector<tsqa_block_group> vg;
    try {
        if (plan_item_ranges(out_start, n_blocks, item_first_block, n_items, ranges, n_ranges, out_cap, vi, vg, &why)) return TSQA_ERR_ARG;
    } catch (...) { return TSQA_ERR_ARG; }
    *n_range_items = (uint32_t)vi.size();
    *n_groups = (uint32_t)vg.size();
    if (vi.size() > cap_items || vg.size() > cap_groups) return TSQA_ERR_ARG;
    std::copy(vi.begin(), vi.end(), items);
    std::copy(vg.begin(), vg.end(), groups);
    return TSQA_OK;
}

extern "C" int tsqa_decompress_item_ranges_async(tsqa_ctx* c, const tsqa_index* idx, const tsqa_item_range* ranges, uint32_t n_ranges,
                                                 void* d_out, size_t out_cap, int32_t* d_status, void* hip_stream)
{
    static_assert(sizeof(tsqa_block_group) == sizeof(BlockGroup) && sizeof(tsqa_item_range) == 32, "public group = kernel group");
    if (!c) return TSQA_ERR_ARG;
    if (!idx || !d_out || !d_status || (n_ranges && !ranges)) { c->set_error("decompress_item_ranges: null pointer"); return TSQA_ERR_ARG; }
    if (idx->device != c->device) { c->set_error("decompress_item_ranges: the index belongs to device %d, the context to %d", idx->device, c->device); return TSQA_ERR_ARG; }
    const char* why = "out of host memory";
    std::vector<tsqa_range_item> vi;
    std::vector<tsqa_block_group> vg;
    int prc = TSQA_ERR_ARG;
    try {
        prc = plan_item_ranges(idx->out_start.data(), idx->n_blocks, idx->item_first.data(), (uint32_t)idx->item_status.size(), ranges, n_ranges,
                               out_cap, vi, vg, &why);
    } catch (...) {}
    if (prc) { c->set_error("decompress_item_ranges: %s", why); return TSQA_ERR_ARG; }
    hipStream_t s = hip_stream ? static_cast<hipStream_t>(hip_stream) : c->stream;
    (void)hipSetDevice(c->device);
    const uint32_t n_items = (uint32_t)vi.size(), n_groups = (uint32_t)vg.size();
    const size_t groups_at = ((size_t)n_items * sizeof(tsqa_range_item) + 15u) & ~(size_t)15u, bytes = groups_at + (size_t)n_groups * sizeof(tsqa_block_group);
    int k = 0;
    if (int rc = c->reserve_upload(c->range_up, bytes ? bytes : 16, &k)) return rc;
    TSQ_HIP(c, hipMemsetAsync(d_status, 0, sizeof(int32_t), s));
    if (n_groups == 0) return TSQA_OK;
    uint8_t* const host = static_cast<uint8_t*>(c->range_up.host[k]);
    memset(host, 0, bytes);
    memcpy(host, vi.data(), (size_t)n_items * sizeof(tsqa_range_item));
    memcpy(host + groups_at, vg.data(), (size_t)n_groups * sizeof(tsqa_block_group));
    TSQ_HIP(c, hipMemcpyAsync(c->range_up.dev[k], host, bytes, hipMemcpyHostToDevice, s));
    const uint8_t* const dev = static_cast<const uint8_t*>(c->range_up.dev[k]);
    const int rc = launch_group_kernel(c, idx->container, idx->frames, idx->n_blocks, reinterpret_cast<const RangeItem*>(dev), n_items,
                                       reinterpret_cast<const BlockGroup*>(dev + groups_at), n_groups, static_cast<uint8_t*>(d_out), d_status, s);
    TSQ_HIP(c, hipEventRecord(c->range_up.done[k], s));
    c->range_up.pending[k] = true;
    if (rc) return rc;
    TSQ_HIP(c, hipGetLastError());
    return TSQA_OK;
}

extern "C" int tsqa_decompress_item_ranges(tsqa_ctx* c, const tsqa_index* idx, const tsqa_item_range* ranges, uint32_t n_ranges, void* d_out,
                                           size_t out_cap, void* hip_stream)
{
    if (!c) return TSQA_ERR_ARG;
    hipStream_t s = hip_stream ? static_cast<hipStream_t>(hip_stream) : c->stream;
    int rc = tsqa_decompress_item_ranges_async(c, idx, ranges, n_ranges, d_out, out_cap, c->d_status, s);
    if (rc) return rc;
    int32_t st = 0;
    TSQ_HIP(c, hipMemcpyAsync(&st, c->d_status, sizeof(st), hipMemcpyDeviceToHost, s));
    TSQ_HIP(c, hipStreamSynchronize(s));
    return status_to_rc(c, st, "decompress_item_ranges");
}


enum BatchPlan { kPlanCompress, kPlanDecompress, kPlanRangesOnly };

static int plan_batch(const tsqa_batch_item* items, uint32_t n_items, size_t in_size, size_t out_size, const uint32_t* n_blocks,
                      uint64_t* first_block, const char** why, BatchPlan mode)
{
    *why = "";
    if (!items || n_items == 0) { *why = "no items"; return TSQA_ERR_ARG; }
    auto blocks_of = [&](uint32_t i) -> uint64_t {
        return mode == kPlanCompress ? items[i].in_len / kBlockSize + (items[i].in_len % kBlockSize != 0) : mode == kPlanDecompress ? n_blocks[i] : 0;
    };
    std::vector<std::pair<uint64_t, uint64_t>> dst;
    dst.reserve(n_items);
    uint64_t blocks = 0;
    for (uint32_t i = 0; i < n_items; ++i) {
        const tsqa_batch_item& x = items[i];
        const uint64_t nb = blocks_of(i);
        if (x.in_len == 0) { *why = "an item is empty"; return TSQA_ERR_ARG; }
        if (x.in_len > in_size || x.in_at > in_size - x.in_len) { *why = "an input range ends past in_size"; return TSQA_ERR_ARG; }
        if (x.out_cap > out_size || x.out_at > out_size - x.out_cap) { *why = "an output range ends past out_size"; return TSQA_ERR_ARG; }
        if (mode == kPlanCompress && x.out_cap < kHeaderSize + kMinFrameSize * nb) { *why = "an output range holds less than 16 + 6 bytes per block"; return TSQA_ERR_ARG; }
        if (mode != kPlanCompress && x.in_len < kHeaderSize) { *why = "an input range is shorter than a header"; return TSQA_ERR_ARG; }
        if (mode == kPlanDecompress && (nb == 0 || nb > (x.in_len - kHeaderSize) / kMinFrameSize)) { *why = "a block count that the container cannot hold"; return TSQA_ERR_ARG; }
        if (x.out_cap) dst.emplace_back(x.out_at, x.out_cap);
        blocks += nb;
    }
    std::sort(dst.begin(), dst.end());
    for (size_t k = 1; k < dst.size(); ++k)
        if (dst[k - 1].first + dst[k - 1].second > dst[k].first) { *why = "two output ranges overlap"; return TSQA_ERR_ARG; }
    if (blocks > 0xFFFFFFFFull) { *why = "more than 2^32 - 1 blocks"; return TSQA_ERR_ARG; }
    if (mode == kPlanRangesOnly) return TSQA_OK;
    uint64_t at = 0;
    for (uint32_t i = 0; i < n_items; ++i) { first_block[i] = at; at += blocks_of(i); }
    first_block[n_items] = at;
    return TSQA_OK;
}

extern "C" int tsqa_plan_batch(const tsqa_batch_item* items, uint32_t n_items, size_t in_size, size_t out_size, const uint32_t* n_blocks,
                               uint64_t* first_block)
{
    const char* why;
    if (!first_block) return TSQA_ERR_ARG;
    return plan_batch(items, n_items, in_size, out_size, n_blocks, first_block, &why, n_blocks ? kPlanDecompress : kPlanCompress);
}

extern "C" int tsqa_compress_batch_async(tsqa_ctx* c, const void* d_in, size_t in_size, const tsqa_batch_item* items, uint32_t n_items,
                                         uint32_t ext, void* d_out, size_t out_size, uint64_t* d_sizes, int32_t* d_status, void* hip_stream)
{
    static_assert(sizeof(tsqa_batch_item) == 32 && sizeof(BatchItem) == 48 && sizeof(EncBatchBlock) == 24, "descriptor layouts");
    if (!c) return TSQA_ERR_ARG;
    if (!d_in || !d_out || !d_sizes || !d_status) { c->set_error("compress_batch: null pointer"); return TSQA_ERR_ARG; }
    const int v = c->enc_variant;
    if (v != 0 && v != 6 && v != 7) { c->set_error("compress_batch: encoder variant %d does not take batches (0, 6 and 7 do)", v); return TSQA_ERR_ARG; }
    std::vector<uint64_t> first((size_t)n_items + 1);
    const char* why;
    if (plan_batch(items, n_items, in_size, out_size, nullptr, first.data(), &why, kPlanCompress)) { c->set_error("compress_batch: %s", why); return TSQA_ERR_ARG; }
    hipStream_t s = hip_stream ? static_cast<hipStream_t>(hip_stream) : c->stream;
    (void)hipSetDevice(c->device);
    const uint64_t n_blocks = first[n_items];
    const uint32_t budget = 2u * (uint32_t)c->n_cus;
    const size_t item_bytes = (size_t)n_items * sizeof(BatchItem), bytes = item_bytes + n_blocks * sizeof(EncBatchBlock);
    int k = 0;
    if (int rc = c->reserve_upload(c->batch_up, bytes, &k)) return rc;
    if (int rc = c->reserve(n_blocks < budget ? n_blocks : budget, true)) return rc;
    if (int rc = c->reserve_batch(n_items)) return rc;
    uint8_t* const host = static_cast<uint8_t*>(c->batch_up.host[k]);
    BatchItem* const hi = reinterpret_cast<BatchItem*>(host);
    EncBatchBlock* const hb = reinterpret_cast<EncBatchBlock*>(host + item_bytes);
    for (uint32_t i = 0; i < n_items; ++i) {
        const tsqa_batch_item& x = items[i];
        const uint32_t nb = (uint32_t)(first[i + 1] - first[i]);
        hi[i] = BatchItem{x.in_at, x.in_len, x.out_at, x.out_cap, first[i], nb, 0u};
        for (uint32_t j = 0; j < nb; ++j) {
            const uint64_t b = first[i] + j, off = (uint64_t)j * kBlockSize, left = x.in_len - off;
            hb[b] = EncBatchBlock{x.in_at + off, left, left < kBlockSize ? (uint32_t)left : kBlockSize, (uint32_t)(b % budget)};
        }
    }
    const BatchItem* const di = static_cast<const BatchItem*>(c->batch_up.dev[k]);
    const EncBatchBlock* const db = reinterpret_cast<const EncBatchBlock*>(static_cast<const uint8_t*>(c->batch_up.dev[k]) + item_bytes);
    const uint8_t* const in = static_cast<const uint8_t*>(d_in);
    uint8_t* const out = static_cast<uint8_t*>(d_out);
    TSQ_HIP(c, hipMemsetAsync(d_status, 0, sizeof(int32_t), s));
    TSQ_HIP(c, hipMemcpyAsync(c->batch_up.dev[k], host, bytes, hipMemcpyHostToDevice, s));
    const uint32_t pieces = (kSlotSize + kPackPiece - 1) / kPackPiece + 1;
    int rc = TSQA_OK;
    for (uint64_t b0 = 0; b0 < n_blocks; b0 += budget) {
        const uint32_t nb = (uint32_t)(n_blocks - b0 < budget ? n_blocks - b0 : budget);
        const uint32_t i0 = (uint32_t)(std::upper_bound(first.begin(), first.end(), b0) - first.begin()) - 1u;
        const uint32_t i1 = (uint32_t)(std::lower_bound(first.begin(), first.begin() + n_items, b0 + nb) - first.begin());
        const bool timed = c->prof_begin(0, s);
        rc = launch_batch_encode_kernels(c, in, db + b0, nb, ext, c->slots, c->sizes, d_status, s);
        if (rc) { if (timed) c->prof_used[0]--; break; }
        if (timed) c->prof_end(0, s);
        hipLaunchKernelGGL(batch_pack_scan_kernel, dim3((i1 - i0 + 255u) / 256u), dim3(256), 0, s, di, i0, i1 - i0, b0, nb, c->sizes, ext, out,
                           c->batch_at, c->frame_at, d_sizes, d_status);
        hipLaunchKernelGGL(batch_pack_copy_kernel, dim3(pieces, nb), dim3(256), 0, s, c->slots, c->sizes, c->frame_at, out);
    }
    TSQ_HIP(c, hipEventRecord(c->batch_up.done[k], s));
    c->batch_up.pending[k] = true;
    if (rc) return rc;
    TSQ_HIP(c, hipGetLastError());
    return TSQA_OK;
}

extern "C" int tsqa_compress_batch(tsqa_ctx* c, const void* d_in, size_t in_size, const tsqa_batch_item* items, uint32_t n_items, uint32_t ext,
                                   void* d_out, size_t out_size, uint64_t* sizes, void* hip_stream)
{
    if (!c) return TSQA_ERR_ARG;
    if (!sizes) { c->set_error("compress_batch: null pointer"); return TSQA_ERR_ARG; }
    hipStream_t s = hip_stream ? static_cast<hipStream_t>(hip_stream) : c->stream;
    if (int rc = c->reserve_batch(n_items)) return rc;
    int rc = tsqa_compress_batch_async(c, d_in, in_size, items, n_items, ext, d_out, out_size, c->batch_sizes, c->d_status, s);
    if (rc) return rc;
    int32_t st = 0;
    TSQ_HIP(c, hipMemcpyAsync(sizes, c->batch_sizes, (size_t)n_items * sizeof(uint64_t), hipMemcpyDeviceToHost, s));
    TSQ_HIP(c, hipMemcpyAsync(&st, c->d_status, sizeof(st), hipMemcpyDeviceToHost, s));
    TSQ_HIP(c, hipStreamSynchronize(s));
    return status_to_rc(c, st, "compress_batch");
}

static int decompress_batch_async_impl(tsqa_ctx* c, const void* d_in, size_t in_size, const tsqa_batch_item* items, const uint32_t* n_blocks,
                                       uint32_t n_items, void* d_out, size_t out_size, uint64_t* d_sizes, int32_t* d_status, hipStream_t s,
                                       int variant)
{
    if (!d_in || !d_out || !d_sizes || !d_status || !n_blocks) { c->set_error("decompress_batch: null pointer"); return TSQA_ERR_ARG; }
    std::vector<uint64_t> first((size_t)n_items + 1);
    const char* why;
    if (plan_batch(items, n_items, in_size, out_size, n_blocks, first.data(), &why, kPlanDecompress)) { c->set_error("decompress_batch: %s", why); return TSQA_ERR_ARG; }
    (void)hipSetDevice(c->device);
    const uint32_t total_blocks = (uint32_t)first[n_items];
    int k = 0;
    if (int rc = c->reserve_upload(c->batch_up, (size_t)n_items * sizeof(BatchItem), &k)) return rc;
    if (int rc = c->reserve(total_blocks, false, false)) return rc;
    c->forget_sharded();
    BatchItem* const hi = static_cast<BatchItem*>(c->batch_up.host[k]);
    for (uint32_t i = 0; i < n_items; ++i)
        hi[i] = BatchItem{items[i].in_at, items[i].in_len, items[i].out_at, items[i].out_cap, first[i], n_blocks[i], 0u};
    TSQ_HIP(c, hipMemsetAsync(d_status, 0, sizeof(int32_t), s));
    TSQ_HIP(c, hipMemcpyAsync(c->batch_up.dev[k], hi, (size_t)n_items * sizeof(BatchItem), hipMemcpyHostToDevice, s));
    hipLaunchKernelGGL(batch_walk_kernel, dim3((n_items + 255u) / 256u), dim3(256), 0, s, static_cast<const uint8_t*>(d_in),
                       static_cast<const BatchItem*>(c->batch_up.dev[k]), n_items, c->frames, d_sizes, d_status);
    const int rc = c->launch_decode_frames(d_in, c->frames, total_blocks, d_out, d_status, s, variant);
    TSQ_HIP(c, hipEventRecord(c->batch_up.done[k], s));
    c->batch_up.pending[k] = true;
    return rc;
}

extern "C" int tsqa_decompress_batch_async(tsqa_ctx* c, const void* d_in, size_t in_size, const tsqa_batch_item* items, const uint32_t* n_blocks,
                                           uint32_t n_items, void* d_out, size_t out_size, uint64_t* d_sizes, int32_t* d_status, void* hip_stream)
{
    if (!c) return TSQA_ERR_ARG;
    hipStream_t s = hip_stream ? static_cast<hipStream_t>(hip_stream) : c->stream;
    return decompress_batch_async_impl(c, d_in, in_size, items, n_blocks, n_items, d_out, out_size, d_sizes, d_status, s, -1);
}

static int decompress_batch_wait(tsqa_ctx* c, const void* d_in, size_t in_size, const tsqa_batch_item* items, const uint32_t* n_blocks,
                                 uint32_t n_items, void* d_out, size_t out_size, uint64_t* sizes, int32_t* st, hipStream_t s)
{
    for (int variant : {-1, 4}) {
        if (int rc = decompress_batch_async_impl(c, d_in, in_size, items, n_blocks, n_items, d_out, out_size, c->batch_sizes, c->d_status, s, variant)) return rc;
        TSQ_HIP(c, hipMemcpyAsync(sizes, c->batch_sizes, (size_t)n_items * sizeof(uint64_t), hipMemcpyDeviceToHost, s));
        TSQ_HIP(c, hipMemcpyAsync(st, c->d_status, sizeof(int32_t), hipMemcpyDeviceToHost, s));
        TSQ_HIP(c, hipStreamSynchronize(s));
        if (*st != kErrStall) break;
    }
    return TSQA_OK;
}

extern "C" int tsqa_decompress_batch(tsqa_ctx* c, const void* d_in, size_t in_size, const tsqa_batch_item* items, uint32_t n_items,
                                     void* d_out, size_t out_size, uint64_t* sizes, int32_t* item_status, void* hip_stream)
{
    if (!c) return TSQA_ERR_ARG;
    if (!d_in || !d_out || !sizes) { c->set_error("decompress_batch: null pointer"); return TSQA_ERR_ARG; }
    const char* why;
    if (plan_batch(items, n_items, in_size, out_size, nullptr, nullptr, &why, kPlanRangesOnly)) { c->set_error("decompress_batch: %s", why); return TSQA_ERR_ARG; }
    hipStream_t s = hip_stream ? static_cast<hipStream_t>(hip_stream) : c->stream;
    (void)hipSetDevice(c->device);
    std::vector<int32_t> own;
    if (!item_status) { own.resize(n_items); item_status = own.data(); }
    if (int rc = c->reserve_batch(n_items)) return rc;
    int k = 0;
    if (int rc = c->reserve_upload(c->batch_up, (size_t)n_items * sizeof(BatchItem), &k)) return rc;
    BatchItem* const hi = static_cast<BatchItem*>(c->batch_up.host[k]);
    for (uint32_t i = 0; i < n_items; ++i) hi[i] = BatchItem{items[i].in_at, items[i].in_len, items[i].out_at, items[i].out_cap, 0, 0, 0};
    std::vector<uint8_t> heads((size_t)n_items * kHeaderSize);
    TSQ_HIP(c, hipMemcpyAsync(c->batch_up.dev[k], hi, (size_t)n_items * sizeof(BatchItem), hipMemcpyHostToDevice, s));
    hipLaunchKernelGGL(batch_heads_kernel, dim3((uint32_t)(((uint64_t)n_items * kHeaderSize + 255u) / 256u)), dim3(256), 0, s,
                       static_cast<const uint8_t*>(d_in), static_cast<const BatchItem*>(c->batch_up.dev[k]), n_items, c->batch_heads);
    TSQ_HIP(c, hipEventRecord(c->batch_up.done[k], s));
    c->batch_up.pending[k] = true;
    TSQ_HIP(c, hipMemcpyAsync(heads.data(), c->batch_heads, heads.size(), hipMemcpyDeviceToHost, s));
    TSQ_HIP(c, hipStreamSynchronize(s));
    std::vector<tsqa_batch_item> ok_items;
    std::vector<uint32_t> ok_blocks, ok_index;
    for (uint32_t i = 0; i < n_items; ++i) {
        sizes[i] = 0;
        uint32_t nb = 0; uint64_t total = 0;
        if (read_header(&heads[(size_t)i * kHeaderSize], items[i].in_len, &nb, &total) != kHeaderOk) item_status[i] = TSQA_ERR_FORMAT;
        else if (total > items[i].out_cap) item_status[i] = TSQA_ERR_ARG;
        else { item_status[i] = TSQA_OK; ok_items.push_back(items[i]); ok_blocks.push_back(nb); ok_index.push_back(i); }
    }
    if (!ok_items.empty()) {
        const uint32_t m = (uint32_t)ok_items.size();
        std::vector<uint64_t> got(m);
        int32_t st = 0;
        if (int rc = decompress_batch_wait(c, d_in, in_size, ok_items.data(), ok_blocks.data(), m, d_out, out_size, got.data(), &st, s)) return rc;
        if (st == 0) {
            for (uint32_t j = 0; j < m; ++j) sizes[ok_index[j]] = got[j];
        } else {
            for (uint32_t j = 0; j < m; ++j) {
                uint64_t one = 0;
                if (int rc = decompress_batch_wait(c, d_in, in_size, &ok_items[j], &ok_blocks[j], 1, d_out, out_size, &one, &st, s)) return rc;
                item_status[ok_index[j]] = st;
                sizes[ok_index[j]] = st ? 0 : one;
            }
        }
    }
    int32_t worst = TSQA_OK;
    uint32_t refused = 0;
    for (uint32_t i = 0; i < n_items; ++i) { worst = std::max(worst, item_status[i]); refused += item_status[i] != TSQA_OK; }
    if (worst) c->set_error("decompress_batch: %u of %u items refused (worst status %d)", refused, n_items, worst);
    return worst;
}


static int index_create_batch(tsqa_ctx* c, const void* d_in, size_t in_size, const tsqa_batch_item* items, uint32_t n_items,
                              tsqa_index** out, int32_t* item_status, tsqa_index** made)
{
    std::vector<tsqa_batch_item> plain;
    if (items && n_items) {
        plain.assign(items, items + n_items);
        for (tsqa_batch_item& x : plain) { x.out_at = 0; x.out_cap = 0; }
    }
    const char* why;
    if (plan_batch(plain.empty() ? nullptr : plain.data(), n_items, in_size, 0, nullptr, nullptr, &why, kPlanRangesOnly)) {
        c->set_error("index_create_batch: %s", why);
        return TSQA_ERR_ARG;
    }
    hipStream_t s = c->stream;
    (void)hipSetDevice(c->device);
    if (int rc = c->reserve_batch(n_items)) return rc;
    const uint8_t* const in = static_cast<const uint8_t*>(d_in);
    int k = 0;
    if (int rc = c->reserve_upload(c->batch_up, (size_t)n_items * sizeof(BatchItem), &k)) return rc;
    BatchItem* hi = static_cast<BatchItem*>(c->batch_up.host[k]);
    for (uint32_t i = 0; i < n_items; ++i) hi[i] = BatchItem{items[i].in_at, items[i].in_len, 0, 0, 0, 0, 0};
    std::vector<uint8_t> heads((size_t)n_items * kHeaderSize);
    TSQ_HIP(c, hipMemcpyAsync(c->batch_up.dev[k], hi, (size_t)n_items * sizeof(BatchItem), hipMemcpyHostToDevice, s));
    hipLaunchKernelGGL(batch_heads_kernel, dim3((uint32_t)(((uint64_t)n_items * kHeaderSize + 255u) / 256u)), dim3(256), 0, s, in,
                       static_cast<const BatchItem*>(c->batch_up.dev[k]), n_items, c->batch_heads);
    TSQ_HIP(c, hipEventRecord(c->batch_up.done[k], s));
    c->batch_up.pending[k] = true;
    TSQ_HIP(c, hipMemcpyAsync(heads.data(), c->batch_heads, heads.size(), hipMemcpyDeviceToHost, s));
    TSQ_HIP(c, hipStreamSynchronize(s));
    std::vector<uint32_t> nbs(n_items);
    std::vector<uint64_t> first((size_t)n_items + 1), verdicts(n_items);
    if (int rc = c->reserve_upload(c->batch_up, (size_t)n_items * sizeof(BatchItem), &k)) return rc;
    hi = static_cast<BatchItem*>(c->batch_up.host[k]);
    uint64_t blocks = 0, cat = 0;
    for (uint32_t i = 0; i < n_items; ++i) {
        uint32_t nb = 0; uint64_t total = 0;
        if (read_header(&heads[(size_t)i * kHeaderSize], items[i].in_len, &nb, &total) != kHeaderOk) { nb = 0; total = 0; }
        nbs[i] = nb; first[i] = blocks;
        hi[i] = BatchItem{items[i].in_at, items[i].in_len, cat, 0, blocks, nb, 0u};
        blocks += nb; cat += total;
    }
    first[n_items] = blocks;
    if (blocks > 0xFFFFFFFFull) { c->set_error("index_create_batch: more than 2^32 - 1 blocks"); return TSQA_ERR_ARG; }
    tsqa_index* idx = new (std::nothrow) tsqa_index();
    if (!idx) { c->set_error("index_create_batch: out of host memory"); return TSQA_ERR_ARG; }
    *made = idx;
    idx->device = c->device; idx->container = in; idx->n = in_size;
    std::vector<tsqa_frame> walked(blocks);
    auto walk = [&]() -> int {
        TSQ_HIP(c, hipMalloc(&idx->frames, (size_t)(blocks ? blocks : 1) * sizeof(FrameInfo)));
        TSQ_HIP(c, hipMemcpyAsync(c->batch_up.dev[k], hi, (size_t)n_items * sizeof(BatchItem), hipMemcpyHostToDevice, s));
        hipLaunchKernelGGL(batch_index_walk_kernel, dim3((n_items + 255u) / 256u), dim3(256), 0, s, in, static_cast<const BatchItem*>(c->batch_up.dev[k]),
                           n_items, idx->frames, c->batch_sizes);
        TSQ_HIP(c, hipGetLastError());
        TSQ_HIP(c, hipEventRecord(c->batch_up.done[k], s));
        c->batch_up.pending[k] = true;
        TSQ_HIP(c, hipMemcpyAsync(verdicts.data(), c->batch_sizes, (size_t)n_items * sizeof(uint64_t), hipMemcpyDeviceToHost, s));
        if (blocks) TSQ_HIP(c, hipMemcpyAsync(walked.data(), idx->frames, (size_t)blocks * sizeof(FrameInfo), hipMemcpyDeviceToHost, s));
        TSQ_HIP(c, hipStreamSynchronize(s));
        return TSQA_OK;
    };
    if (int rc = walk()) return rc;
    idx->item_first.resize((size_t)n_items + 1);
    idx->item_status.resize(n_items);
    bool gaps = false;
    uint64_t total = 0;
    int32_t worst = TSQA_OK;
    uint32_t refused = 0;
    for (uint32_t i = 0; i < n_items; ++i) {
        const bool ok = verdicts[i] != kItemRefused;
        idx->item_first[i] = idx->host_frames.size();
        idx->item_status[i] = ok ? TSQA_OK : TSQA_ERR_FORMAT;
        if (item_status) item_status[i] = idx->item_status[i];
        if (!ok) { gaps |= nbs[i] != 0u; refused++; worst = TSQA_ERR_FORMAT; continue; }
        for (uint64_t b = first[i]; b < first[i + 1]; ++b) {
            tsqa_frame f = walked[b];
            f.out_at = total;
            idx->out_start.push_back(total);
            idx->host_frames.push_back(f);
            total += f.out_len;
        }
    }
    idx->item_first[n_items] = idx->host_frames.size();
    idx->out_start.push_back(total);
    idx->n_blocks = (uint32_t)idx->host_frames.size();
    idx->total = total;
    if (gaps && idx->n_blocks) {
        const hipError_t e = hipMemcpy(idx->frames, idx->host_frames.data(), (size_t)idx->n_blocks * sizeof(FrameInfo), hipMemcpyHostToDevice);
        if (e != hipSuccess) { c->set_error("index_create_batch: hipMemcpy failed: %s", hipGetErrorString(e)); return TSQA_ERR_HIP; }
    }
    if (worst) c->set_error("index_create_batch: %u of %u items refused", refused, n_items);
    *out = idx;
    return worst;
}

extern "C" int tsqa_index_create_batch(tsqa_ctx* c, const void* d_in, size_t in_size, const tsqa_batch_item* items, uint32_t n_items,
                                       tsqa_index** out, int32_t* item_status)
{
    if (!out) return TSQA_ERR_ARG;
    *out = nullptr;
    if (!c) return TSQA_ERR_ARG;
    if (!d_in) { c->set_error("index_create_batch: null pointer"); return TSQA_ERR_ARG; }
    tsqa_index* made = nullptr;
    int rc;
    try { rc = index_create_batch(c, d_in, in_size, items, n_items, out, item_status, &made); }
    catch (...) { c->set_error("index_create_batch: out of host memory"); rc = TSQA_ERR_ARG; *out = nullptr; }
    if (!*out) tsqa_index_destroy(made);
    return rc;
}

typedef uint32_t probe_u32x4 __attribute__((ext_vector_type(4)));
template <int MODE>
__global__ __launch_bounds__(256) void copy_probe_kernel(const probe_u32x4* __restrict__ src, probe_u32x4* __restrict__ dst, size_t words)
{
    if (MODE == 2) {
        const size_t i = (size_t)blockIdx.x * 1024u + threadIdx.x;
        if (i + 768u < words) {
            const probe_u32x4 a = __builtin_nontemporal_load(src + i), b = __builtin_nontemporal_load(src + i + 256), c = __builtin_nontemporal_load(src + i + 512),
                                d = __builtin_nontemporal_load(src + i + 768);
            __builtin_nontemporal_store(a, dst + i); __builtin_nontemporal_store(b, dst + i + 256);
            __builtin_nontemporal_store(c, dst + i + 512); __builtin_nontemporal_store(d, dst + i + 768);
        } else for (size_t k = i; k < words && k < i + 1024u; k += 256u) dst[k] = src[k];
        return;
    }
    const size_t step = (size_t)gridDim.x * 256u;
    size_t i = (size_t)blockIdx.x * 256u + threadIdx.x;
    for (; i + 3 * step < words; i += 4 * step) {
        if (MODE == 1) {
            const probe_u32x4 a = __builtin_nontemporal_load(src + i), b = __builtin_nontemporal_load(src + i + step), c = __builtin_nontemporal_load(src + i + 2 * step),
                                d = __builtin_nontemporal_load(src + i + 3 * step);
            __builtin_nontemporal_store(a, dst + i); __builtin_nontemporal_store(b, dst + i + step);
            __builtin_nontemporal_store(c, dst + i + 2 * step); __builtin_nontemporal_store(d, dst + i + 3 * step);
        } else {
            const probe_u32x4 a = src[i], b = src[i + step], c = src[i + 2 * step], d = src[i + 3 * step];
            dst[i] = a; dst[i + step] = b; dst[i + 2 * step] = c; dst[i + 3 * step] = d;
        }
    }
    for (; i < words; i += step) dst[i] = src[i];
}

extern "C" int tsqa_measure_copy(tsqa_ctx* c, size_t bytes, int reps, double* best_gbps, double* median_gbps)
{
    if (!c || bytes < (size_t(1) << 20) || reps < 1 || reps > 64) return TSQA_ERR_ARG;
    (void)hipSetDevice(c->device);
    probe_u32x4 *a = nullptr, *b = nullptr;
    hipEvent_t e0 = nullptr, e1 = nullptr;
    const size_t words = bytes / 16;
    int rc = TSQA_OK;
    double rates[64];
    if (hipMalloc(&a, words * 16) != hipSuccess || hipMalloc(&b, words * 16) != hipSuccess ||
        hipEventCreate(&e0) != hipSuccess || hipEventCreate(&e1) != hipSuccess ||
        hipMemsetAsync(a, 0x5a, words * 16, c->stream) != hipSuccess) rc = TSQA_ERR_HIP;
    uint32_t grid = (uint32_t)c->n_cus * 8u;
    int mode = 0;
    auto launch = [&](int m, uint32_t g) {
        if (m == 0) hipLaunchKernelGGL(copy_probe_kernel<0>, dim3(g), dim3(256), 0, c->stream, a, b, words);
        else if (m == 1) hipLaunchKernelGGL(copy_probe_kernel<1>, dim3(g), dim3(256), 0, c->stream, a, b, words);
        else hipLaunchKernelGGL(copy_probe_kernel<2>, dim3((uint32_t)((words + 1023u) / 1024u)), dim3(256), 0, c->stream, a, b, words);
    };
    {
        float best_ms = 1e30f;
        for (int m = 0; m < 3 && rc == TSQA_OK; ++m)
            for (uint32_t per_cu = 8; per_cu <= (m == 2 ? 8u : 64u) && rc == TSQA_OK; per_cu *= 2) {
                const uint32_t g = (uint32_t)c->n_cus * per_cu;
                float ms = 1e30f;
                for (int k = 0; k < 2; ++k) {
                    (void)hipEventRecord(e0, c->stream);
                    launch(m, g);
                    (void)hipEventRecord(e1, c->stream);
                    if (hipEventSynchronize(e1) != hipSuccess || hipEventElapsedTime(&ms, e0, e1) != hipSuccess) { rc = TSQA_ERR_HIP; break; }
                }
                if (ms < best_ms) { best_ms = ms; grid = g; mode = m; }
            }
    }
    for (int r = -1; r < reps && rc == TSQA_OK; ++r) {
        (void)hipEventRecord(e0, c->stream);
        launch(mode, grid);
        (void)hipEventRecord(e1, c->stream);
        float ms = 0;
        if (hipEventSynchronize(e1) != hipSuccess || hipEventElapsedTime(&ms, e0, e1) != hipSuccess || ms <= 0) { rc = TSQA_ERR_HIP; break; }
        if (r >= 0) rates[r] = 2.0 * (double)(words * 16) / (ms * 1e-3) / 1e9;
    }
    if (rc == TSQA_OK) {
        for (int i = 1; i < reps; ++i) for (int j = i; j > 0 && rates[j] < rates[j - 1]; --j) { double t = rates[j]; rates[j] = rates[j - 1]; rates[j - 1] = t; }
        if (best_gbps) *best_gbps = rates[reps - 1];
        if (median_gbps) *median_gbps = rates[reps / 2];
        snprintf(c->probe_shape, sizeof(c->probe_shape), "copy probe: mode %d (0 grid-stride, 1 grid-stride non-temporal, 2 one pass non-temporal), %u workgroups", mode, mode == 2 ? (uint32_t)((words + 1023u) / 1024u) : grid);
    } else c->set_error("copy probe failed");
    if (e0) (void)hipEventDestroy(e0);
    if (e1) (void)hipEventDestroy(e1);
    (void)hipFree(a); (void)hipFree(b);
    return rc;
}

extern "C" const char* tsqa_copy_probe_shape(const tsqa_ctx* c) { return c ? c->probe_shape : ""; }

#ifdef TSQ_SPINS
extern "C" int tsqa_debug_spins(uint32_t* out16)
{
    return hipMemcpyFromSymbol(out16, HIP_SYMBOL(tsq::g_enc_spins), 20 * sizeof(uint32_t)) == hipSuccess ? TSQA_OK : TSQA_ERR_HIP;
}
#endif
#if defined(TSQ_STATS) || defined(TSQ_TRACEONLY)
extern "C" int tsqa_debug_trace(uint32_t* out4096)
{
    return hipMemcpyFromSymbol(out4096, HIP_SYMBOL(tsq::g_enc_trace), 4096 * sizeof(uint32_t)) == hipSuccess ? TSQA_OK : TSQA_ERR_HIP;
}
#endif
#ifdef TSQ_STATS
extern "C" int tsqa_debug_stats(unsigned long long* enc64, unsigned long long* dec16)
{
    if (enc64 && hipMemcpyFromSymbol(enc64, HIP_SYMBOL(tsq::g_enc_stats), 64 * sizeof(unsigned long long)) != hipSuccess) return TSQA_ERR_HIP;
    if (dec16 && hipMemcpyFromSymbol(dec16, HIP_SYMBOL(tsq::g_dec_stats), 16 * sizeof(unsigned long long)) != hipSuccess) return TSQA_ERR_HIP;
    return TSQA_OK;
}
extern "C" int tsqa_debug_dec_waves(unsigned long long* out48)
{
    return hipMemcpyFromSymbol(out48, HIP_SYMBOL(tsq::g_dec_wave), 48 * sizeof(unsigned long long)) == hipSuccess ? TSQA_OK : TSQA_ERR_HIP;
}
extern "C" int tsqa_debug_duo_xcc(uint32_t* out2048)
{
    return hipMemcpyFromSymbol(out2048, HIP_SYMBOL(tsq::g_duo_xcc), 2048 * sizeof(uint32_t)) == hipSuccess ? TSQA_OK : TSQA_ERR_HIP;
}
extern "C" int tsqa_debug_syms(uint32_t* out8192)
{
    return hipMemcpyFromSymbol(out8192, HIP_SYMBOL(tsq::g_dbg_syms), 8192 * sizeof(uint32_t)) == hipSuccess ? TSQA_OK : TSQA_ERR_HIP;
}
#endif
```

Measured before the change: 22.78.

## Replace LDS ring-history decoder with far-history kernel reading old output from global

After: 22.50. 1.2% lower.

```diff
diff --git a/turbosqueeze_amd/csrc/tsq_dec_common.cuh b/turbosqueeze_amd/csrc/tsq_dec_common.cuh
--- a/turbosqueeze_amd/csrc/tsq_dec_common.cuh
+++ b/turbosqueeze_amd/csrc/tsq_dec_common.cuh
@@ -38,6 +38,29 @@
 static_assert(SymCfg::MAXG <= SymCfg::T / 2 && SymCfg::MAXG % SymCfg::HOP == 0 && SymCfg::MAXG >= SymCfg::S / 13 + 2 * SymCfg::HOP, "group table");
 static_assert(4 * SymCfg::MAXG <= 2 * SymCfg::T, "at most two pairs per lane");
 
+template <class C>
+struct Geo {
+    static constexpr uint32_t BPL = C::OUTC / C::T;
+    static constexpr uint32_t PB = C::S + C::SPAD <= 8192u ? 13u : 14u;
+    static constexpr uint32_t VMASK = (1u << (30u - PB)) - 1u;
+    static constexpr uint32_t REPS = (4u * C::MAXG + C::T - 1u) / C::T;
+    static_assert(BPL * C::T == C::OUTC && BPL % 4u == 0u, "whole words per lane");
+    static_assert(C::S + C::SPAD <= (1u << PB) && C::OUTC <= VMASK, "pair word");
+    static_assert(C::OUTC + 16u <= 0x8000u, "a byte entry is 0x8000 | value or the index of another entry");
+    static_assert(C::MAXG <= C::T && C::MAXG % C::HOP == 0 && C::MAXG >= C::S / 13 + 2 * C::HOP && C::MAXSN * C::HOP <= C::T, "one lane per group");
+    static_assert(C::S % C::T == 0 && C::SWORDS <= C::T && C::R % 16 == 0, "lane counts, ring phase");
+};
+template <class C, class = void>
+struct WaitList {
+    static_assert(64u * Geo<C>::BPL == 768u, "twelve bytes per lane");
+    static __device__ __forceinline__ uint32_t at(uint32_t wid) { return 768u * wid; }
+};
+template <class C>
+struct WaitList<C, std::void_t<decltype(C::WL)>> {
+    static_assert(C::WL == 64u * Geo<C>::BPL, "one entry per byte of the wavefront");
+    static __device__ __forceinline__ uint32_t at(uint32_t wid) { return C::WL * wid; }
+};
+
 __device__ __forceinline__ void pair_lens(uint32_t sb, uint32_t cc, uint32_t ext, uint32_t& slen, uint32_t& olen)
 {
     const uint32_t hi = sb >> 4, lo = sb & 15u;
@@ -54,9 +77,9 @@
     __device__ __forceinline__ uint32_t a0() const { return at & ~3u; }
 };
 
+template <class C = SymCfg>
 __device__ __forceinline__ uint4 prefetch_words(const uint8_t* in, uint32_t at, uint32_t av)
 {
-    using C = SymCfg;
     const uint32_t tid = threadIdx.x;
     const uint32_t lim = av < C::S + C::SPAD ? av : C::S + C::SPAD;
     uint4 w = make_uint4(0, 0, 0, 0);
@@ -66,7 +89,7 @@
 template <class L>
 __device__ __forceinline__ void stage_words(uint8_t* lds, const uint8_t* in, uint32_t at, uint32_t av, uint4 pre)
 {
-    using C = SymCfg;
+    using C = typename L::C;
     const uint32_t tid = threadIdx.x;
     if (tid < C::SWORDS) {
         uint4 w = pre;
@@ -81,9 +104,9 @@
 }
 
 template <class L>
-__device__ __forceinline__ void parse_groups(uint8_t* lds, uint32_t slim, uint32_t (&x)[SymCfg::PER])
-{
-    using C = SymCfg;
+__device__ __forceinline__ void parse_groups(uint8_t* lds, uint32_t slim, uint32_t (&x)[L::C::PER])
+{
+    using C = typename L::C;
     const uint32_t tid = threadIdx.x;
     const uint8_t* const sbuf = lds + L::sbuf;
     uint32_t y[C::PER], c[C::PER];
@@ -125,9 +148,9 @@
 }
 
 template <class L>
-__device__ __forceinline__ void double_pointers(uint8_t* lds, uint32_t slim, uint32_t (&x)[SymCfg::PER])
-{
-    using C = SymCfg;
+__device__ __forceinline__ void double_pointers(uint8_t* lds, uint32_t slim, uint32_t (&x)[L::C::PER])
+{
+    using C = typename L::C;
     const uint32_t tid = threadIdx.x;
     const uint8_t* const j1 = lds + L::j1;
     uint16_t* const j2 = reinterpret_cast<uint16_t*>(lds + L::j2);
@@ -157,7 +180,7 @@
 template <class L>
 __device__ __forceinline__ uint32_t walk_chain(uint8_t* lds, uint32_t first, uint32_t slim)
 {
-    using C = SymCfg;
+    using C = typename L::C;
     const uint16_t* const j16 = reinterpret_cast<const uint16_t*>(lds + L::j16);
     uint16_t* const sn = reinterpret_cast<uint16_t*>(lds + L::sn);
     uint32_t* const misc = reinterpret_cast<uint32_t*>(lds + L::misc);
@@ -179,7 +202,7 @@
 template <class L>
 __device__ __forceinline__ void group_lanes(uint8_t* lds, uint32_t nsn, uint32_t slim, uint32_t op, uint32_t size, uint32_t ext)
 {
-    using C = SymCfg;
+    using C = typename L::C;
     const uint32_t tid = threadIdx.x, lane = tid & 63u, wid = tid >> 6;
     const uint8_t* const sbuf = lds + L::sbuf;
     const uint8_t* const j1 = lds + L::j1;
@@ -209,7 +232,7 @@
 #pragma unroll
         for (uint32_t pr = 0; pr < 4; ++pr) {
             const uint32_t cc = (c >> (6u - 2u * pr)) & 3u;
-            pw[pr] = p | (v << 13) | (cc << 30);
+            pw[pr] = p | (v << Geo<C>::PB) | (cc << 30);
             uint32_t sl, ol;
             pair_lens(sbuf[p], cc, ext, sl, ol);
             p += sl;
@@ -252,17 +275,21 @@
     return {ng, misc[5], ng ? gout[ng - 1] + glen[ng - 1] : op, false, false};
 }
 
+struct RingHistory {
+    static constexpr bool kFar = false;
+};
 template <class L>
 __device__ __forceinline__ void clear_records(uint8_t* lds)
 {
     uint32_t* const recw = reinterpret_cast<uint32_t*>(lds + L::recw);
-    for (uint32_t w = threadIdx.x; w < (SymCfg::OUTC + 16) / 4; w += SymCfg::T) *reinterpret_cast<uint4*>(recw + 4u * w) = make_uint4(0, 0, 0, 0);
-}
-template <class L, class PairAt>
+    using C = typename L::C;
+    for (uint32_t w = threadIdx.x; w < (C::OUTC + 16) / 4; w += C::T) *reinterpret_cast<uint4*>(recw + 4u * w) = make_uint4(0, 0, 0, 0);
+}
+template <class L, class PairAt, class H = RingHistory>
 __device__ __forceinline__ void drop_records(uint8_t* lds, uint32_t ng, const Image& im, uint32_t size, uint32_t avail, uint32_t ext,
-                                             PairAt pair_at)
-{
-    using C = SymCfg;
+                                             PairAt pair_at, H hist = H())
+{
+    using C = typename L::C;
     const uint32_t tid = threadIdx.x;
     const uint8_t* const sbuf = lds + L::sbuf;
     uint32_t* const recw = reinterpret_cast<uint32_t*>(lds + L::recw);
@@ -270,12 +297,12 @@
     if (tid == 0 && lead) recw[0] = 0x40000000u | (L::ring + a0);
     uint32_t bad = 0;
 #pragma unroll
-    for (uint32_t rep = 0; rep < 2; ++rep) {
+    for (uint32_t rep = 0; rep < Geo<C>::REPS; ++rep) {
         const uint32_t gi = tid + rep * C::T;
         if (gi >= ng * 4u) break;
         const uint2 pg = pair_at(rep, gi);
         const uint32_t pw = pg.x;
-        uint32_t p = pw & 0x1FFFu, j = pg.y + ((pw >> 13) & 0x3FFFu);
+        uint32_t p = pw & ((1u << Geo<C>::PB) - 1u), j = pg.y + ((pw >> Geo<C>::PB) & Geo<C>::VMASK);
         const uint32_t origin = j;
         uint32_t sb = 0;
         if (j < size) { if (p >= avail) bad = 1; sb = sbuf[p]; p++; }
@@ -301,11 +328,17 @@
                     if (!bad) {
                         const uint32_t a = origin - off;
                         const uint32_t n_hist = a >= op ? 0u : (op - a < take ? op - a : take);
-                        if (n_hist) {
-                            uint32_t x0 = a0 + C::R - ((op - a) - lead);
+                        uint32_t n_far = 0;
+                        if constexpr (H::kFar) {
+                            n_far = a >= hist.near_lo ? 0u : (hist.near_lo - a < take ? hist.near_lo - a : take);
+                            if (n_far) hist.far(lds, recw, 2u * rep + sidx, gi >> 2, a, n_far, ij);
+                        }
+                        if (n_hist > n_far) {
+                            const uint32_t ir = ij + n_far, nr = n_hist - n_far;
+                            uint32_t x0 = a0 + C::R - ((op - (a + n_far)) - lead);
                             x0 -= x0 >= C::R ? C::R : 0u;
-                            recw[ij] = 0x40000000u | ((L::ring + x0 - ij) & 0xFFFFFFu);
-                            if (x0 + n_hist > C::R) { const uint32_t n1 = C::R - x0; recw[ij + n1] = 0x40000000u | ((L::ring - (ij + n1)) & 0xFFFFFFu); }
+                            recw[ir] = 0x40000000u | ((L::ring + x0 - ir) & 0xFFFFFFu);
+                            if (x0 + nr > C::R) { const uint32_t n1 = C::R - x0; recw[ir + n1] = 0x40000000u | ((L::ring - (ir + n1)) & 0xFFFFFFu); }
                         }
                         if (n_hist < take) recw[ij + n_hist] = 0xC0000000u | ((a - j) & 0xFFFFFFu);
                     }
@@ -314,6 +347,7 @@
             }
         }
     }
+    if constexpr (H::kFar) hist.finish(lds);
     if (bad) reinterpret_cast<uint32_t*>(lds + L::misc)[4] = kErrStream;
 }
 
@@ -322,45 +356,49 @@
 template <class L>
 __device__ __forceinline__ uint32_t fetch_bytes(uint8_t* lds, const Image& im)
 {
+    using C = typename L::C;
+    constexpr uint32_t B = Geo<C>::BPL;
     const uint32_t tid = threadIdx.x, lane = tid & 63u, wid = tid >> 6;
     const uint32_t* const recw = reinterpret_cast<const uint32_t*>(lds + L::recw);
     uint32_t* const wsum = reinterpret_cast<uint32_t*>(lds + L::wsum);
-    lds_u16* const wl = (lds_u16*)(lds + L::plist) + 768u * wid;
-    const uint32_t own = 12u * tid;
-    uint32_t r[12];
+    lds_u16* const wl = (lds_u16*)(lds + L::plist) + WaitList<C>::at(wid);
+    const uint32_t own = B * tid;
+    uint32_t r[B];
     {
-        const uint4 q0 = *reinterpret_cast<const uint4*>(recw + own), q1 = *reinterpret_cast<const uint4*>(recw + own + 4u),
-                    q2 = *reinterpret_cast<const uint4*>(recw + own + 8u);
-        r[0] = q0.x; r[1] = q0.y; r[2] = q0.z; r[3] = q0.w; r[4] = q1.x; r[5] = q1.y; r[6] = q1.z; r[7] = q1.w; r[8] = q2.x; r[9] = q2.y; r[10] = q2.z; r[11] = q2.w;
-#pragma unroll
-        for (uint32_t k = 1; k < 12; ++k) r[k] = r[k] ? r[k] : r[k - 1];
-        const uint32_t upto = wave_scan_last(r[11]);
+#pragma unroll
+        for (uint32_t w = 0; w < B / 4u; ++w) {
+            const uint4 q = *reinterpret_cast<const uint4*>(recw + own + 4u * w);
+            r[4 * w] = q.x; r[4 * w + 1] = q.y; r[4 * w + 2] = q.z; r[4 * w + 3] = q.w;
+        }
+#pragma unroll
+        for (uint32_t k = 1; k < B; ++k) r[k] = r[k] ? r[k] : r[k - 1];
+        const uint32_t upto = wave_scan_last(r[B - 1]);
         uint32_t carry = (uint32_t)__builtin_amdgcn_update_dpp(0, (int)upto, 0x138, 0xF, 0xF, false);
         if (lane == 63) wsum[wid] = upto;
         __syncthreads();
         {
-            const uint32_t ws = lane < 16u ? wsum[lane] : 0u;
+            const uint32_t ws = lane < C::T / 64u ? wsum[lane] : 0u;
             const uint64_t m = __ballot(ws != 0u && lane < wid);
             const uint32_t prev = m ? (uint32_t)__builtin_amdgcn_readlane((int)ws, 63 - __builtin_clzll(m)) : 0u;
             carry = carry ? carry : prev;
         }
 #pragma unroll
-        for (uint32_t k = 0; k < 12; ++k) r[k] = r[k] ? r[k] : carry;
+        for (uint32_t k = 0; k < B; ++k) r[k] = r[k] ? r[k] : carry;
     }
     uint32_t pend = 0;
     if (own < im.lead() + im.len) {
-        uint32_t v[12], by[12];
-#pragma unroll
-        for (uint32_t k = 0; k < 12; ++k) {
+        uint32_t v[B], by[B];
+#pragma unroll
+        for (uint32_t k = 0; k < B; ++k) {
             v[k] = own + k + (uint32_t)((int32_t)(r[k] << 8) >> 8);
             pend |= (r[k] >> 31) << k;
         }
 #pragma unroll
-        for (uint32_t k = 0; k < 12; ++k) by[k] = lds[(r[k] >> 31) ? 0u : v[k]];
-#pragma unroll
-        for (uint32_t k = 0; k < 12; ++k) v[k] = (r[k] >> 31) ? v[k] : (0x8000u | by[k]);
-#pragma unroll
-        for (uint32_t w = 0; w < 3; ++w)
+        for (uint32_t k = 0; k < B; ++k) by[k] = lds[(r[k] >> 31) ? 0u : v[k]];
+#pragma unroll
+        for (uint32_t k = 0; k < B; ++k) v[k] = (r[k] >> 31) ? v[k] : (0x8000u | by[k]);
+#pragma unroll
+        for (uint32_t w = 0; w < B / 4u; ++w)
             *reinterpret_cast<uint2*>(lds + L::ent + 2u * own + 8u * w) = make_uint2(v[4 * w] | (v[4 * w + 1] << 16), v[4 * w + 2] | (v[4 * w + 3] << 16));
     }
     const uint32_t cnt = (uint32_t)__builtin_popcount(pend);
@@ -368,7 +406,7 @@
     const uint32_t n_wait = (uint32_t)__builtin_amdgcn_readlane((int)incl, 63);
     uint32_t at = incl - cnt;
 #pragma unroll
-    for (uint32_t k = 0; k < 12; ++k) {
+    for (uint32_t k = 0; k < B; ++k) {
         if ((pend >> k) & 1u) wl[at] = (uint16_t)(own + k);
         at += (pend >> k) & 1u;
     }
@@ -378,13 +416,15 @@
 template <class L>
 __device__ __forceinline__ uint32_t jump_pointers(uint8_t* lds, uint32_t n_wait)
 {
+    using C = typename L::C;
+    constexpr uint32_t B = Geo<C>::BPL;
     const uint32_t lane = threadIdx.x & 63u, wid = threadIdx.x >> 6;
     lds_u16* const le = (lds_u16*)(lds + L::ent);
-    lds_u16* const wl = (lds_u16*)(lds + L::plist) + 768u * wid;
-    const uint32_t spare = SymCfg::OUTC + wid;
+    lds_u16* const wl = (lds_u16*)(lds + L::plist) + WaitList<C>::at(wid);
+    const uint32_t spare = C::OUTC + wid;
     if (lane == 0) le[spare] = 0x8000u;
     const uint32_t passes = (n_wait + 63u) >> 6;
-    const uint32_t padded = passes <= 2u ? 2u : passes <= 4u ? 4u : passes <= 6u ? 6u : passes <= 8u ? 8u : 12u;
+    const uint32_t padded = passes <= 2u ? 2u : passes <= 4u ? 4u : passes <= 6u ? 6u : passes <= 8u ? 8u : passes <= 12u ? 12u : B;
     if (passes) for (uint32_t it = n_wait + lane; it < padded * 64u; it += 64u) wl[it] = (uint16_t)spare;
     uint32_t iters = 0;
     auto jump = [&](auto passes_c) {
@@ -413,21 +453,26 @@
     else if (passes <= 4u) jump(std::integral_constant<uint32_t, 4>{});
     else if (passes <= 6u) jump(std::integral_constant<uint32_t, 6>{});
     else if (passes <= 8u) jump(std::integral_constant<uint32_t, 8>{});
-    else jump(std::integral_constant<uint32_t, 12>{});
+    else if (B == 12u || passes <= 12u) jump(std::integral_constant<uint32_t, 12>{});
+    else jump(std::integral_constant<uint32_t, B>{});
     return iters;
 }
 
 template <class L>
 __device__ __forceinline__ void write_ring(uint8_t* lds, const Image& im)
 {
-    using C = SymCfg;
-    const uint32_t own = 12u * threadIdx.x;
+    using C = typename L::C;
+    constexpr uint32_t B = Geo<C>::BPL;
+    const uint32_t own = B * threadIdx.x;
     if (own >= im.lead() + im.len) return;
-    const uint2 e0 = *reinterpret_cast<const uint2*>(lds + L::ent + 2u * own), e1 = *reinterpret_cast<const uint2*>(lds + L::ent + 2u * own + 8u),
-                e2 = *reinterpret_cast<const uint2*>(lds + L::ent + 2u * own + 16u);
-    const uint32_t ev[6] = {e0.x, e0.y, e1.x, e1.y, e2.x, e2.y};
-#pragma unroll
-    for (uint32_t w = 0; w < 3; ++w) {
+    uint32_t ev[B / 2u];
+#pragma unroll
+    for (uint32_t w = 0; w < B / 4u; ++w) {
+        const uint2 e = *reinterpret_cast<const uint2*>(lds + L::ent + 2u * own + 8u * w);
+        ev[2 * w] = e.x; ev[2 * w + 1] = e.y;
+    }
+#pragma unroll
+    for (uint32_t w = 0; w < B / 4u; ++w) {
         uint32_t x = im.a0() + own + 4u * w; x -= x >= C::R ? C::R : 0u;
         const uint32_t lo = ev[2 * w], hi = ev[2 * w + 1];
         *reinterpret_cast<uint32_t*>(lds + L::ring + x) = (lo & 0xFFu) | ((lo >> 8) & 0xFF00u) | ((hi & 0xFFu) << 16) | ((hi >> 16) << 24);
@@ -437,7 +482,7 @@
 template <class L>
 __device__ __forceinline__ void flush_image(const uint8_t* lds, uint8_t* out, const Image& im, uint32_t first_tid, uint32_t n_threads)
 {
-    using C = SymCfg;
+    using C = typename L::C;
     const uint32_t tid = threadIdx.x;
     const uint8_t* const ring = lds + L::ring;
     if (im.len == 0 || tid < first_tid) return;
@@ -459,7 +504,7 @@
 __device__ __forceinline__ void flush_window(const uint8_t* lds, uint8_t* out, const Image& im, uint32_t lo, uint32_t hi, uint32_t first_tid,
                                              uint32_t n_threads)
 {
-    using C = SymCfg;
+    using C = typename L::C;
     const uint32_t a = im.op > lo ? im.op : lo, b = im.op + im.len < hi ? im.op + im.len : hi;
     if (a >= b) return;
     uint32_t at = im.at + (a - im.op); at -= at >= C::R ? C::R : 0u;
diff --git a/turbosqueeze_amd/csrc/tsq_dec_duo.cuh b/turbosqueeze_amd/csrc/tsq_dec_duo.cuh
--- a/turbosqueeze_amd/csrc/tsq_dec_duo.cuh
+++ b/turbosqueeze_amd/csrc/tsq_dec_duo.cuh
@@ -151,6 +151,7 @@
 }
 
 struct DuoCopyLds {
+    using C = SymCfg;
     static constexpr uint32_t sbuf = 0;
     static constexpr uint32_t recw = sbuf + 16 * SymCfg::SWORDS;
     static constexpr uint32_t ent = recw;
diff --git a/turbosqueeze_amd/csrc/tsq_dec_hist.cuh b/turbosqueeze_amd/csrc/tsq_dec_hist.cuh
--- /dev/null
+++ b/turbosqueeze_amd/csrc/tsq_dec_hist.cuh
@@ -0,0 +1,210 @@
+#pragma once
+
+#include "tsq_common.cuh"
+#include "tsq_dec_common.cuh"
+#include "tsq_experiment.h"
+
+#ifndef TSQ_HIST_S
+#define TSQ_HIST_S 8192
+#endif
+#ifndef TSQ_HIST_NSLOT
+#define TSQ_HIST_NSLOT 2048
+#endif
+
+namespace tsq {
+
+struct HistCfg {
+    static constexpr uint32_t T = 1024;
+    static constexpr uint32_t S = TSQ_HIST_S;
+    static constexpr uint32_t SPAD = 160;
+    static constexpr uint32_t OUTC = 2 * S;
+    static constexpr uint32_t HOP = 16;
+    static constexpr uint32_t MAXG = (S / 13 + 2 * HOP + HOP - 1) / HOP * HOP;
+    static constexpr uint32_t MAXSN = MAXG / HOP + 2;
+    static constexpr uint32_t PER = S / T;
+    static constexpr uint32_t TERM = S + SPAD;
+    static constexpr uint32_t R = OUTC + 128;
+    static constexpr uint32_t RPAD = 64;
+    static constexpr uint32_t SWORDS = (S + SPAD + 16) / 16;
+    static constexpr uint32_t WL = 64 * (OUTC / T);
+    static constexpr uint32_t NSLOT = TSQ_HIST_NSLOT;
+    static constexpr uint32_t FAR_MIN = 16;
+};
+static_assert(HistCfg::NSLOT >= 32, "one group alone (eight symbols of four pieces) always finds its slots");
+
+struct HistLds {
+    using C = HistCfg;
+    static constexpr uint32_t sbuf = 0;
+    static constexpr uint32_t j1 = sbuf + 16 * C::SWORDS;
+    static constexpr uint32_t JN = (C::S + C::SPAD + 8u) & ~7u;
+    static constexpr uint32_t j2 = j1 + C::S;
+    static constexpr uint32_t j4 = j2 + 2 * JN;
+    static constexpr uint32_t j8 = j4 + 2 * JN;
+    static constexpr uint32_t j16 = j8 + 2 * JN;
+    static constexpr uint32_t recw = j1;
+    static constexpr uint32_t ent = j1;
+    static constexpr uint32_t plist = ent + 2 * (C::OUTC + 16);
+    static constexpr uint32_t gstart = j16 + 2 * JN;
+    static constexpr uint32_t glen = gstart + 2 * C::MAXG;
+    static constexpr uint32_t gout = glen + 2 * C::MAXG;
+    static constexpr uint32_t pairs = gout + 4 * C::MAXG;
+    static constexpr uint32_t sn = pairs + 16 * C::MAXG;
+    static constexpr uint32_t wsum = (sn + 2 * ((C::MAXSN + 7) & ~7u) + 15) & ~15u;
+    static constexpr uint32_t misc = wsum + 64;
+    static constexpr uint32_t slots = (misc + 64 + 15) & ~15u;
+    static constexpr uint32_t ring = slots + 16 * C::NSLOT;
+    static constexpr uint32_t total = ring + C::R + C::RPAD;
+    static_assert(recw % 16 == 0 && recw + 4 * (C::OUTC + 16) <= gstart && plist % 16 == 0 && plist + 2 * 16 * C::WL <= gstart,
+                  "records, byte entries and waiting lists fit the dead doubling tables");
+};
+static_assert(HistLds::total <= 160 * 1024, "LDS budget");
+
+template <class L>
+struct FarHistory {
+    using C = typename L::C;
+    typedef uint32_t u32x4 __attribute__((ext_vector_type(4)));
+    static constexpr bool kFar = true;
+    static constexpr uint32_t K = 2u * Geo<C>::REPS;
+    uint32_t near_lo = 0;
+    __amdgpu_buffer_rsrc_t rsrc;
+    u32x4 held[K];
+    uint32_t held_at[K] = {};
+
+    __device__ __forceinline__ u32x4 load(uint32_t pos, uint32_t& at) const
+    {
+        at = pos + 16u <= near_lo ? pos : near_lo - 16u;
+#ifdef TSQ_X_HIST_FIXED
+        return __builtin_amdgcn_raw_buffer_load_b128(rsrc, 0, 0, 16);
+#else
+        return __builtin_amdgcn_raw_buffer_load_b128(rsrc, (int)at, 0, 16);
+#endif
+    }
+    __device__ __forceinline__ void far(uint8_t* lds, uint32_t* recw, uint32_t k, uint32_t grp, uint32_t a, uint32_t n, uint32_t ij)
+    {
+        uint32_t* const misc = reinterpret_cast<uint32_t*>(lds + L::misc);
+        const uint64_t m = __ballot(1);
+        const uint32_t rank = __builtin_amdgcn_mbcnt_hi((uint32_t)(m >> 32), __builtin_amdgcn_mbcnt_lo((uint32_t)m, 0u));
+        uint32_t base = 0;
+        if (rank == 0u) base = atomicAdd(&misc[6], (uint32_t)__builtin_popcountll(m));
+        const uint32_t s0 = (uint32_t)__builtin_amdgcn_readfirstlane((int)base) + rank;
+        const uint32_t extra = (n - 1u) >> 4;
+        const uint32_t s1 = extra ? atomicAdd(&misc[6], extra) : 0u;
+        if (s0 >= C::NSLOT || s1 + extra > C::NSLOT) { atomicMin(&misc[7], grp); return; }
+        uint32_t at;
+        held[k] = load(a, at);
+        held_at[k] = L::slots + 16u * s0;
+        recw[ij] = 0x40000000u | ((L::slots + 16u * s0 + (a - at) - ij) & 0xFFFFFFu);
+        for (uint32_t q = 0; q < extra; ++q) {
+            const uint32_t pos = a + 16u * (q + 1u), iq = ij + 16u * (q + 1u), sa = L::slots + 16u * (s1 + q);
+            *reinterpret_cast<u32x4*>(lds + sa) = load(pos, at);
+            recw[iq] = 0x40000000u | ((sa + (pos - at) - iq) & 0xFFFFFFu);
+        }
+    }
+    __device__ __forceinline__ void finish(uint8_t* lds)
+    {
+#pragma unroll
+        for (uint32_t k = 0; k < K; ++k)
+            if (held_at[k]) *reinterpret_cast<u32x4*>(lds + held_at[k]) = held[k];
+    }
+};
+
+__global__ __launch_bounds__(1024) void dec_hist_kernel(const uint8_t* __restrict__ container, const FrameInfo* __restrict__ frames,
+                                                        uint8_t* __restrict__ outbuf, int32_t* __restrict__ status)
+{
+    using C = HistCfg;
+    using L = HistLds;
+    extern __shared__ __attribute__((aligned(16))) uint8_t lds[];
+    const uint16_t* const gstart = reinterpret_cast<const uint16_t*>(lds + L::gstart);
+    const uint32_t* const gout = reinterpret_cast<const uint32_t*>(lds + L::gout);
+    const uint32_t* const pairs = reinterpret_cast<const uint32_t*>(lds + L::pairs);
+    uint32_t* const misc = reinterpret_cast<uint32_t*>(lds + L::misc);
+
+    const uint32_t tid = threadIdx.x;
+    if (tid == 0) misc[11] = (uint32_t)*status;
+    __syncthreads();
+    if (misc[11] != 0u) return;
+    const FrameInfo f = frames[blockIdx.x];
+    if (f.stream_len < 3u || f.stream_len > kSlotSize || f.out_len > kBlockSize) {
+        if (tid == 0) atomicMax(status, kErrStream);
+        return;
+    }
+    const uint8_t* const in = container + f.stream_at;
+    uint8_t* const out = outbuf + f.out_at;
+    const uint32_t in_len = f.stream_len, size = f.out_len, ext = f.ext;
+    const uint32_t oskew = (uint32_t)((uintptr_t)out & 15u);
+
+    if (tid == 0) misc[4] = 0;
+    uint32_t sp = 3, op = 0;
+    uint32_t ring_op = oskew;
+    Image prev = {0, 0, 0};
+    uint4 pre = prefetch_words<C>(in, sp, in_len - sp);
+    bool staged_ahead = false;
+    __syncthreads();
+
+    while (op < size) {
+        const uint32_t avail = in_len - sp;
+        const uint32_t slim = avail < C::S ? avail : C::S;
+        if (!staged_ahead) stage_words<L>(lds, in, sp, avail, pre);
+        if (tid == 0) { misc[0] = 0; misc[1] = 0; misc[2] = 0xFFFFFFFFu; misc[3] = 0xFFFFFFFFu; misc[5] = 0; misc[6] = 0; misc[7] = 0xFFFFFFFFu; }
+        __syncthreads();
+
+        uint32_t x[C::PER];
+        parse_groups<L>(lds, slim, x);
+        double_pointers<L>(lds, slim, x);
+        const uint32_t nsn = walk_chain<L>(lds, 0u, slim);
+
+        if (tid >= C::T / 2) flush_image<L>(lds, out, prev, C::T / 2, C::T / 2);
+        group_lanes<L>(lds, nsn, slim, op, size, ext);
+        clear_records<L>(lds);
+        __syncthreads();
+        ChunkEnd e = chunk_end<L>(lds, op, size);
+        uint32_t next_sp = sp + e.next_at;
+        if (misc[4] != 0 || e.ng == 0 || (!e.last && next_sp >= in_len)) {
+            if (tid == 0) atomicMax(status, kErrStream);
+            return;
+        }
+        Image im = {op, e.next_op - op, ring_op};
+        bool more = !e.last;
+        if (more) pre = prefetch_words<C>(in, next_sp, in_len - next_sp);
+
+        FarHistory<L> hist;
+        hist.near_lo = prev.op >= C::FAR_MIN ? prev.op : 0u;
+        hist.rsrc = __builtin_amdgcn_make_buffer_rsrc(out, 0, (int)hist.near_lo, 0x00020000);
+        const auto pair_at = [&](uint32_t, uint32_t gi) { return make_uint2(pairs[gi], gout[gi >> 2]); };
+        drop_records<L>(lds, e.ng, im, size, avail, ext, pair_at, hist);
+        __syncthreads();
+        if (misc[4] != 0) { if (tid == 0) atomicMax(status, (int32_t)misc[4]); return; }
+        if (misc[7] != 0xFFFFFFFFu) {
+            const uint32_t cutg = misc[7] ? misc[7] : 1u;
+            e = ChunkEnd{cutg, gstart[cutg], gout[cutg], false, true};
+            next_sp = sp + e.next_at;
+            im = Image{op, e.next_op - op, ring_op};
+            more = true;
+            pre = prefetch_words<C>(in, next_sp, in_len - next_sp);
+            __syncthreads();
+            if (tid == 0) { misc[6] = 0; misc[7] = 0xFFFFFFFFu; }
+            clear_records<L>(lds);
+            __syncthreads();
+            drop_records<L>(lds, e.ng, im, size, avail, ext, pair_at, hist);
+            __syncthreads();
+            if (misc[4] != 0 || misc[7] != 0xFFFFFFFFu) { if (tid == 0) atomicMax(status, kErrStream); return; }
+        }
+        const uint32_t n_wait = fetch_bytes<L>(lds, im);
+        __syncthreads();
+        if (more) { stage_words<L>(lds, in, next_sp, in_len - next_sp, pre); staged_ahead = true; }
+        asm volatile("s_waitcnt vmcnt(0)" ::: "memory");
+        jump_pointers<L>(lds, n_wait);
+        __syncthreads();
+        write_ring<L>(lds, im);
+
+        prev = im;
+        ring_op += im.len; ring_op -= ring_op >= C::R ? C::R : 0u;
+        op = e.next_op;
+        sp = next_sp;
+        if (!more) break;
+    }
+    __syncthreads();
+    flush_image<L>(lds, out, prev, 0, C::T);
+}
+
+}
diff --git a/turbosqueeze_amd/csrc/tsq_dec_sym.cuh b/turbosqueeze_amd/csrc/tsq_dec_sym.cuh
--- a/turbosqueeze_amd/csrc/tsq_dec_sym.cuh
+++ b/turbosqueeze_amd/csrc/tsq_dec_sym.cuh
@@ -6,6 +6,7 @@
 namespace tsq {
 
 struct SymLds {
+    using C = SymCfg;
     static constexpr uint32_t sbuf = 0;
     static constexpr uint32_t j1 = sbuf + 16 * SymCfg::SWORDS;
     static constexpr uint32_t JN = (SymCfg::S + SymCfg::SPAD + 8u) & ~7u;
diff --git a/turbosqueeze_amd/csrc/tsq_experiment.h b/turbosqueeze_amd/csrc/tsq_experiment.h
--- a/turbosqueeze_amd/csrc/tsq_experiment.h
+++ b/turbosqueeze_amd/csrc/tsq_experiment.h
@@ -1,7 +1,7 @@
 #pragma once
 
 #if defined(TSQ_X_NOHAZ) || defined(TSQ_X_NOCOMMITWAIT) || defined(TSQ_X_NOPATCH) || defined(TSQ_X_FAKE_TABLE) || defined(TSQ_X_FAKE_CAND) || \
-    defined(TSQ_X_FREE_QUERY)
+    defined(TSQ_X_FREE_QUERY) || defined(TSQ_X_HIST_FIXED)
 #define TSQ_TIMING_ONLY_BUILD 1
 #ifndef TSQ_EXPERIMENT
 #error "a timing-only switch (TSQ_X_*: wrong streams on purpose) needs -DTSQ_EXPERIMENT; the product library is never built with one (tools/xbuild.sh)"
diff --git a/turbosqueeze_amd/csrc/tsq_launch.cuh b/turbosqueeze_amd/csrc/tsq_launch.cuh
--- a/turbosqueeze_amd/csrc/tsq_launch.cuh
+++ b/turbosqueeze_amd/csrc/tsq_launch.cuh
@@ -7,6 +7,7 @@
 #include "tsq_internal.h"
 #include "tsq_serial.cuh"
 #include "tsq_dec_sym.cuh"
+#include "tsq_dec_hist.cuh"
 #include "tsq_dec_duo.cuh"
 #include "tsq_enc_stage.cuh"
 #ifdef TSQ_AB_VARIANTS
@@ -113,11 +114,23 @@
 {
     static std::atomic<uint64_t> attr_devices{0};
     {
-        const void* const fns[1] = {reinterpret_cast<const void*>(dec_sym_kernel)};
-        const uint32_t bytes[1] = {SymLds::total};
+        const void* const fns[1] = {reinterpret_cast<const void*>(dec_hist_kernel)};
+        const uint32_t bytes[1] = {HistLds::total};
         if (int rc = raise_lds_limit(c, attr_devices, fns, bytes)) return rc;
     }
     const int v = variant >= 0 ? variant : c->dec_variant;
+#ifdef TSQ_AB_VARIANTS
+    if (v == 7) {
+        static std::atomic<uint64_t> ab_devices{0};
+        const void* const fns[1] = {reinterpret_cast<const void*>(dec_sym_kernel)};
+        const uint32_t bytes[1] = {SymLds::total};
+        if (int rc = raise_lds_limit(c, ab_devices, fns, bytes)) return rc;
+        hipLaunchKernelGGL(dec_sym_kernel, dim3(n_blocks), dim3(SymCfg::T), SymLds::total, s, container, frames, out, status);
+        return 0;
+    }
+#else
+    if (v == 7) { c->set_error("kernel variant %d lives in the A/B library only (make ab)", v); return TSQA_ERR_ARG; }
+#endif
     if (v == 1) { hipLaunchKernelGGL(dec_serial_kernel, dim3(n_blocks), dim3(64), 0, s, container, frames, out, status); return 0; }
     if (v == 8 || v == 9) { c->set_error("kernel variant %d is not built", v); return TSQA_ERR_ARG; }
     auto launch_multi = [&](const FrameInfo* fr, uint32_t nblk, bool three) -> int {
@@ -139,11 +152,11 @@
     if (v == 0 && n_blocks > cus) {
         const uint32_t tail = n_blocks % cus, full = n_blocks - tail;
         if (tail != 0u && 2u * tail <= cus) {
-            hipLaunchKernelGGL(dec_sym_kernel, dim3(full), dim3(SymCfg::T), SymLds::total, s, container, frames, out, status);
+            hipLaunchKernelGGL(dec_hist_kernel, dim3(full), dim3(HistCfg::T), HistLds::total, s, container, frames, out, status);
             return launch_multi(frames + full, tail, 3u * tail <= cus);
         }
     }
-    hipLaunchKernelGGL(dec_sym_kernel, dim3(n_blocks), dim3(SymCfg::T), SymLds::total, s, container, frames, out, status);
+    hipLaunchKernelGGL(dec_hist_kernel, dim3(n_blocks), dim3(HistCfg::T), HistLds::total, s, container, frames, out, status);
     return 0;
 }
 
diff --git a/turbosqueeze_amd/csrc/tsq_runtime.hip b/turbosqueeze_amd/csrc/tsq_runtime.hip
--- a/turbosqueeze_amd/csrc/tsq_runtime.hip
+++ b/turbosqueeze_amd/csrc/tsq_runtime.hip
@@ -64,6 +64,9 @@
 #endif
 #ifdef TSQ_X_FREE_QUERY
            " TSQ_X_FREE_QUERY"
+#endif
+#ifdef TSQ_X_HIST_FIXED
+           " TSQ_X_HIST_FIXED"
 #endif
 #ifdef TSQ_X_DELAY_STAGE
            " TSQ_X_DELAY_STAGE"
```
